# slobodaapl/nvit

Measured on AMD Instinct MI355X. Metric: images/sec (train step) nViT-B/16 224px, higher is better.
Workload: dtype bf16; 1 GPU; nViT-base 224px patches 8/16 T=784 C=768 L=12 H=12, full train step (fwd+bwd+clip+AdamW+renorm), synthetic images, formula weights; per_gpu_batch=128, global_batch=128, parallelism=dp1

## Files before the change

include/nvit_hip.h:

```cpp
#ifndef NVIT_HIP_H
#define NVIT_HIP_H
#include <stdint.h>

#ifdef __cplusplus
extern "C" {
#endif

#define NVIT_OK 0
#define NVIT_EINVAL 1001
#define NVIT_F32 0
#define NVIT_BF16 1
#define NVIT_BF16_F32IN 3

int nvit_version(void);
const char* nvit_last_error(void);

#define NVIT_KID_GEMM_NT 0
#define NVIT_KID_GEMM_TN 1
#define NVIT_KID_ATTN_FWD 2
#define NVIT_KID_ATTN_BWD 3
#define NVIT_KID_ROWOPS 4
#define NVIT_KID_RENORM 5
#define NVIT_KID_SHADOW 6
#define NVIT_KID_PATCHIFY 7
#define NVIT_KID_MISC 8
#define NVIT_KID_GEMM_F32 9
#define NVIT_KID_GEMM_SWIGLU 10
#define NVIT_KID_GEMM_QKNORM 11
#define NVIT_KID_GEMM_SWIGLU_BWD 12
#define NVIT_KID_OPTIM 13
#define NVIT_KID_GEMM_SWIGLU_ACT 14
#define NVIT_KID_COUNT 15
void nvit_prof_enable(int on);
void nvit_prof_select(unsigned mask);
int nvit_prof_collect(double* ms, double* flops, double* bytes, int64_t* launches);
const char* nvit_prof_name(int kid);

#define NVIT_RENORM_ROWS_PER_ITEM 64
#define NVIT_RENORM_COLS_PER_ITEM 64
#define NVIT_RENORM_TALL_ROWS 1152
#define NVIT_RENORM_TALL_COLS_PER_ITEM 32
#define NVIT_RENORM_MAX_ROWS_DIM0 2048
#define NVIT_RENORM_MAX_GRID 2048
int nvit_renorm_weights(const int64_t* table, int n, int total_items, void* stream);

#define NVIT_SHADOW_TILE 64
int nvit_shadow_weights(const int64_t* table, int n, int total_items, int dt, void* stream);

#define NVIT_OPT_TABLE_COLS 10
#define NVIT_OPT_CHUNK 8192
#define NVIT_OPT_ROWS_PER_ITEM 16
#define NVIT_OPT_SLAB_COLS 32
#define NVIT_OPT_SLAB_ROWS 1152
#define NVIT_OPT_TALL_COLS 16
#define NVIT_OPT_TALL_ROWS 2048
#define NVIT_OPT_ROW_COLS 1536
#define NVIT_OPT_WIDE_COLS 2048
#define NVIT_OPT_WIDE_LDS_ROWS 1024
#define NVIT_OPT_MAX_PART 4096
#define NVIT_OPT_MAX_GRID 2048
int nvit_adamw_tick(float* hyper, double beta1, double beta2, void* stream);
int nvit_grad_sqnorm(const int64_t* table, int n, int total_chunks, float* partial, int npart, void* stream);
int nvit_adamw_renorm(const int64_t* table, int n, int total_items, int max_slab_rows, float beta1, float beta2,
                      float eps, double bias_correction1, double bias_correction2, const float* partial, int npart,
                      float max_norm, float* gnorm_out, const float* hyper, void* stream);
int nvit_adamw_tick_guarded(float* hyper, double beta1, double beta2, const float* partial, int npart,
                            float* skip_state, void* stream);
int nvit_adamw_renorm_guarded(const int64_t* table, int n, int total_items, int max_slab_rows, float beta1, float beta2,
                              float eps, const float* partial, int npart, float max_norm, float* gnorm_out,
                              const float* hyper, const float* skip_state, void* stream);
#define NVIT_LR_COSINE 0
#define NVIT_LR_LINEAR 1
#define NVIT_LR_CONSTANT 2
#define NVIT_LR_SCHEDULE_THREADS 256
int nvit_lr_schedule(int64_t* table, int n, const float* lr_scale, int64_t* step, int kind, double lr, double min_lr,
                     double warmup_init, int64_t warmup_iters, int64_t decay_iters, float* last_lr, double* last_lr64,
                     void* stream);

#define NVIT_EMA_TABLE_COLS 5
#define NVIT_EMA_CHUNK 4096
#define NVIT_EMA_MAX_GRID 2048
#define NVIT_EMA_FLAG_COPY 1
#define NVIT_EMA_FLAG_SCALAR 2
int nvit_ema_tick(float* state, double decay, int warmup, const float* skip_state, void* stream);
int nvit_ema_update(const int64_t* table, int n, int total_chunks, const float* state, void* stream);

int nvit_gemm_nt(int dt, const void* A, int lda, const void* B, int ldb, void* C, int ldc, int out_dt,
                 int M, int N, int K, const float* bias, const float* colscale, const float* rowadd,
                 int rowadd_period, int accumulate, void* stream);

#define NVIT_SWIGLU_BWD_TILE_ROWS 256
#define NVIT_SWIGLU_BWD_PART_ROWS 128
int nvit_set_gemm_sched(int dynamic);
int nvit_set_gemm_impl(int nt_impl, int tn_impl);
int nvit_gemm_nt_fusable(int dt, int M, int N, int K);
int nvit_gemm_nt_swiglu_bwd(int dt, const void* A, int lda, const void* B, int ldb, const void* uv, void* duv,
                            float* part, int M, int F, int K, const float* gs, float gscale, void* stream);
int nvit_gemm_nt_swiglu(int dt, const void* A, int lda, const void* B, int ldb, void* uv, void* xm, int M, int F,
                        int K, const float* gs, float gscale, void* stream);
int nvit_gemm_nt_swiglu_act(int dt, const void* A, int lda, const void* B, int ldb, void* xm, int M, int F, int K,
                            const float* gs, float gscale, void* stream);
int nvit_gemm_nt_qknorm(int dt, const void* A, int lda, const void* B, int ldb, int M, int K, int nparts, int part0,
                        const float* sqk, float c_q, float q_prescale, void* qh, void* kh, void* vh, float* rq, float* rk,
                        int T, int H, int d, void* stream);
int nvit_gemm_nt_swiglu_bias(int dt, const void* A, int lda, const void* B, int ldb, void* uv, void* xm, int M, int F,
                             int K, const float* gs, float gscale, const float* bias, void* stream);
int nvit_gemm_nt_swiglu_act_bias(int dt, const void* A, int lda, const void* B, int ldb, void* xm, int M, int F, int K,
                                 const float* gs, float gscale, const float* bias, void* stream);
int nvit_gemm_nt_qknorm_bias(int dt, const void* A, int lda, const void* B, int ldb, int M, int K, int nparts, int part0,
                             const float* sqk, float c_q, float q_prescale, void* qh, void* kh, void* vh, float* rq,
                             float* rk, int T, int H, int d, const float* bias, void* stream);

int nvit_gemm_tn(int dt, const void* A, int lda, const void* B, int ldb, float* G, int ldg, int Mred, int N,
                 int K, int splits, float* ws, int64_t ws_bytes, int perm, int accumulate, void* stream);

#define NVIT_MAX_EMBD 2048
#define NVIT_MAX_PART_BLOCKS 4096
#define NVIT_ROW_WAVES 4
#define NVIT_ROW_GRID_MAX 2048
int nvit_lerp_fwd(int dt, const float* h, const void* y, int y_dt, const float* alpha, float c_a,
                  const float* skip_x, const float* skip, float* out, void* out_lo, int M, int C, void* stream);
int nvit_lerp_bwd_blocks(int dt, int y_dt, int C, int has_add, int has_skip, int accum);
int nvit_lerp_bwd(int dt, const float* dout, const void* dout_add, const float* h, const void* y, int y_dt, const float* alpha,
                  float c_a, const float* skip_x, const float* skip, float* dh, int accum_dh, float* dy,
                  void* dy_lo, float* dskip_x, float* part_dlam, float* part_dskip, int nblk, int M, int C,
                  void* stream);
int nvit_lerp_fwd_gated(int dt, const float* h, const void* y, int y_dt, const float* alpha, float c_a,
                        const float* skip_x, const float* skip, const float* gate, int rows_per_sample, float* out,
                        void* out_lo, int M, int C, void* stream);
int nvit_lerp_bwd_gated_blocks(int dt, int y_dt, int C, int has_add, int has_skip, int accum);
int nvit_lerp_bwd_gated(int dt, const float* dout, const void* dout_add, const float* h, const void* y, int y_dt,
                        const float* alpha, float c_a, const float* skip_x, const float* skip, const float* gate,
                        int rows_per_sample, float* dh, int accum_dh, float* dy, void* dy_lo, float* dskip_x,
                        float* part_dlam, float* part_dskip, int nblk, int M, int C, void* stream);

int nvit_rmsnorm_fwd(const float* x, const float* w, float eps, float* out, float* rstd, int M, int C, void* stream);
int nvit_rmsnorm_bwd(const float* dout, const float* x, const float* w, const float* rstd, float* dx, float* part_dw,
                     int nblk, int M, int C, void* stream);
int nvit_res_rmsnorm_fwd(int dt, const float* a, const void* y, int y_dt, const float* w, float eps, float* out,
                         void* out_lo, float* rstd, int M, int C, void* stream);
int nvit_res_rmsnorm_bwd(int dt, const float* g, const void* g_add, const float* a, const void* y, int y_dt,
                         const float* w, const float* rstd, float* dz, int accum, void* dz_lo, float* part_dw, int nblk,
                         int M, int C, void* stream);
int nvit_res_skip_fwd(int dt, const float* h, const void* y, int y_dt, const float* skip, const float* x, float* out,
                      void* out_lo, int M, int C, void* stream);
int nvit_res_skip_bwd(int dt, const float* dout, const float* h, const void* y, int y_dt, const float* skip,
                      const float* x, float* dh, void* dh_lo, float* dx, float* part_dskip, int nblk, int M, int C,
                      void* stream);
int nvit_res_rmsnorm_fwd_gated(int dt, const float* a, const void* y, int y_dt, const float* w, float eps, const float* gate,
                               int rows_per_sample, float* out, void* out_lo, float* rstd, int M, int C, void* stream);
int nvit_res_rmsnorm_bwd_gated(int dt, const float* g, const void* g_add, const float* a, const void* y, int y_dt,
                               const float* w, const float* rstd, const float* gate, int rows_per_sample, float* dz,
                               int accum, void* dz_lo, float* part_dw, int nblk, int M, int C, void* stream);
int nvit_res_skip_fwd_gated(int dt, const float* h, const void* y, int y_dt, const float* skip, const float* x,
                            const float* gate, int rows_per_sample, float* out, void* out_lo, int M, int C, void* stream);
int nvit_res_skip_bwd_gated(int dt, const float* dout, const float* h, const void* y, int y_dt, const float* skip,
                            const float* x, const float* gate, int rows_per_sample, float* dh, void* dh_lo, float* dx,
                            float* part_dskip, int nblk, int M, int C, void* stream);
int nvit_norm_skip_fwd(const float* src, const float* tgt, const float* skip, float* out, int M, int C, void* stream);
int nvit_norm_skip_bwd(const float* dout, const float* src, const float* tgt, const float* skip, float* dsrc,
                       float* dtgt, float* part_dskip, int nblk, int M, int C, void* stream);

int nvit_qknorm_fwd(int dt, const void* q, int ldq, const void* k, int ldk, const void* v, int ldv,
                    const float* sqk, float c_q, void* qh, void* kh, void* vh, float* rq, float* rk, int B,
                    int T, int H, int d, void* stream);
int nvit_qknorm_bwd(int dt, const void* dqh, const void* dkh, const void* dvh, const void* qh, const void* kh,
                    const float* rq, const float* rk, const float* sqk, float c_q, void* dq, int ldq,
                    void* dk, int ldk, void* dv, int ldv, float* part_dsqk, int nblk, int B, int T, int H,
                    int d, void* stream);

#define NVIT_PAD_HEAD_DIM 128
int nvit_heads_pad_fwd(int dt, const float* q, int ldq, const float* k, int ldk, const float* v, int ldv,
                       const float* sqk, float c_q, void* qh, void* kh, void* vh, float* rq, float* rk,
                       float* sqk_pad, int B, int T, int H, int d, int dp, void* stream);
int nvit_heads_pad_bwd(int dt, const void* dqh, const void* dkh, const void* dvh, const void* qh, const void* kh,
                       const float* rq, const float* rk, const float* sqk, float c_q, void* dq, int ldq,
                       void* dk, int ldk, void* dv, int ldv, float* part_dsqk, int nblk, int B, int T, int H,
                       int d, int dp, void* stream);
int nvit_pad_cols(int dt, const void* src, void* dst, int M, int H, int d, int dp, void* stream);
int nvit_unpad_cols(int dt, const void* src, void* dst, int M, int H, int d, int dp, void* stream);

int nvit_swiglu_fwd(int dt, const void* uv, const float* suv, float gscale, void* x, int M, int F, void* stream);
int nvit_swiglu_bwd(int dt, const void* dx, const void* uv, const float* suv, float gscale, void* duv,
                    float* part_dsuv, int rows_per_blk, int M, int F, void* stream);

int nvit_colsum_reduce(const float* part, int nblk, int N, float* out, int accumulate, int kind, const float* ref,
                       float scale, void* stream);
#define NVIT_COLSUM_REDUCE_MAX_ITEMS 8
int nvit_colsum_reduce_multi(const int64_t* part, const int* nblk, const int64_t* part_b, const int* nblk_b, const int* N,
                             const int64_t* out, const int* accumulate, const int* kind, const int64_t* ref,
                             const float* scale, int n, void* stream);
int nvit_colsum(const void* a, int a_dt, int lda, const void* b, int b_dt, int ldb, int R, int N, int period,
                float* out, int accumulate, float scale, void* stream);
int nvit_cast(const float* src, void* dst, int dt, int64_t n, void* stream);
int nvit_normalize_images(const void* in, int in_is_u8_hwc, float* out, int B, int C, int H, int W, float mean, float std_,
                          void* stream);
#define NVIT_AUG_ROW 8
#define NVIT_AUG_NOPS 15
#define NVIT_AUG_NMAG 10
#define NVIT_AUG_MAX_SIDE 4096
int nvit_augment_draw(const int* policy, int P, uint64_t seed, int64_t* step, int64_t first_index, const int* argtab,
                      int* params, int B, void* stream);
int nvit_augment_apply(const void* in, const int* params, float* out_f32, void* out_u8, void* ws, int64_t ws_bytes, int B,
                       int H, int W, int C, float mean, float std_, void* stream);
#define NVIT_RA_ROW 16
#define NVIT_RA_NCHOICES 15
#define NVIT_RA_SOLARIZE_ADD 15
#define NVIT_RA_NOPS 16
#define NVIT_RA_MAX_LAYERS 4
#define NVIT_RA_ROT_KNOTS 1024
#define NVIT_RA_BILINEAR 0
#define NVIT_RA_BICUBIC 1
#define NVIT_RA_RANDOM 2
int nvit_randaug_draw(uint64_t seed, int64_t* step, int64_t first_index, const double* q, const double* rot, double magnitude,
                      double mstd, double mmax, int increasing, float prob, int interp, double translate_pct, int* params,
                      int B, int num_layers, int H, int W, void* stream);
int nvit_randaug_apply(const void* in, const int* params, float* out_f32, void* out_u8, void* ws, int64_t ws_bytes, int B,
                       int H, int W, int C, int num_layers, int fill0, int fill1, int fill2, float mean, float std_,
                       void* stream);
#define NVIT_MIX_ROW 8
#define NVIT_MIX_KNOTS 1024
int nvit_mix_draw(uint64_t seed, int64_t* step, int64_t first_index, const float* q_mix, const float* q_cut, float prob,
                  float switch_prob, const int64_t* labels, int* table, float* lam, int64_t* y2, int B, int H, int W,
                  void* stream);
int nvit_mix_apply(const float* in, const int* table, float* out, int B, int C, int H, int W, void* stream);
#define NVIT_DROPPATH_MAX_GATES 1048576
int nvit_droppath_draw(uint64_t seed, int64_t* step, int64_t first_index, const float* rates, int scale_by_keep,
                       float* table, int n_layer, int B, void* stream);
#define NVIT_PATCHDROP_MAX_TOKENS 4096
int nvit_patchdrop_draw(uint64_t seed, int64_t* step, int64_t first_index, int* keep, int* slot, int B, int T, int K,
                        void* stream);
int nvit_rows_gather(const float* src0, const float* src1, const int* keep, float* dst0, float* dst1, void* lo0, void* lo1,
                     int lo_dt, int B, int T, int K, int C, void* stream);
int nvit_rows_scatter(const float* d0, const float* d1, const int* slot, float* g0, float* g1, int B, int T, int K, int C,
                      void* stream);
#define NVIT_POS_RESAMPLE_MAX_TAPS 32
#define NVIT_POS_RESAMPLE_MAX_GRID 1024
int nvit_pos_resample_fwd(const float* p0, const float* p1, const int* taps, float* out0, float* out1, int g, int g2, int C,
                          void* stream);
int nvit_pos_resample_bwd(const float* d0, const float* d1, const int* taps_t, float* g0, float* g1, int g, int g2, int C,
                          void* stream);
#define NVIT_CROP_ROW 8
#define NVIT_CROP_KNOTS 1024
#define NVIT_CROP_ATTEMPTS 10
#define NVIT_CROP_MAX_SRC 2048
#define NVIT_CROP_MAX_BATCH 65535
#define NVIT_CROP_BILINEAR 0
#define NVIT_CROP_BICUBIC 1
int nvit_crop_draw(uint64_t seed, int64_t* step, int64_t first_index, const double* aspect, double scale0, double scale1,
                   double ratio_min, double ratio_max, float hflip, int* table, int B, int Hs, int Ws, void* stream);
int64_t nvit_crop_ws_bytes(int B, int Hs, int Ws, int C, int size, int interp);
int nvit_crop_apply(const void* in, const int* table, void* out, void* ws, int64_t ws_bytes, int B, int Hs, int Ws, int C,
                    int size, int interp, void* stream);
#define NVIT_ERASE_ROW 8
#define NVIT_ERASE_KNOTS 1024
#define NVIT_ERASE_CONST 0
#define NVIT_ERASE_PIXEL 1
int nvit_erase_draw(uint64_t seed, int64_t* step, int64_t first_index, const double* aspect, double area0, double area1,
                    float prob, int* table, int B, int H, int W, void* stream);
int nvit_erase_apply(const float* in, const int* table, const float* q, float* out, int mode, int B, int C, int H, int W,
                     void* stream);
int nvit_scale_cols(const float* a, int lda, const float* s, float c, void* out, int out_dt, int ldo, int R, int N,
                    void* stream);

int nvit_attn_fwd(int dt, int impl, const void* qh, const void* kh, const void* vh, float scale, void* o, float* lse,
                  int B, int H, int Tq, int Tk, int d, void* stream);
int nvit_attn_fwd_bounded(int dt, int impl, const void* qh, const void* kh, const void* vh, float scale, const float* sqk,
                          float c_q, float q_prescale, void* o, float* lse, int B, int H, int Tq, int Tk, int d,
                          void* stream);
int nvit_attn_bwd(int dt, int impl, const void* dout, const void* qh, const void* kh, const void* vh, const void* o,
                  const float* lse, float scale, void* dqh, void* dkh, void* dvh, float* delta, int B, int H,
                  int Tq, int Tk, int d, void* stream);

#define NVIT_ATTN_BWD_PART_ROWS 128
int nvit_attn_bwd_qknorm(int dt, const void* dout, const void* qh, const void* kh, const void* vh, const void* o,
                         const float* lse, float scale, const float* rq, const float* rk, const float* sqk, float c_q,
                         float q_prescale, void* dq, int ldq, void* dk, void* dv, int ldkv, float* part_q, float* part_k,
                         float* delta, int B, int H, int Tq, int Tk, int d, void* stream);

// ... 77 lines not shown
```

nvit_amd/_lib.py:

```python
from __future__ import annotations

import ctypes as C
import os
import re

_HERE = os.path.dirname(os.path.abspath(__file__))
LIB_PATH = os.environ.get("NVIT_LIB") or os.path.join(_HERE, "libnvit_hip.so")
HEADER_PATH = os.path.join(os.path.dirname(_HERE), "include", "nvit_hip.h")


def _header_constants() -> dict:
    try:
        with open(HEADER_PATH) as f:
            return {name: int(value) for name, value in re.findall(r"#define NVIT_(\w+)\s+(-?\d+)", f.read())}
    except OSError as e:
        raise ImportError(f"nvit_amd: cannot read the C header that holds the kernels' layout constants: {e}") from None


HEADER = _header_constants()


def const(name: str) -> int:
    if name not in HEADER:
        raise ImportError(f"nvit_amd: {HEADER_PATH} has no integer `#define NVIT_{name}`")
    return HEADER[name]


F32, BF16, BF16_F32IN = 0, 1, 3
KID_NAMES = ["gemm_nt", "gemm_tn", "attn_fwd", "attn_bwd", "rowops", "renorm", "shadow", "patchify", "misc", "gemm_f32",
             "gemm_swiglu", "gemm_qknorm", "gemm_swiglu_bwd", "optim", "gemm_swiglu_act"]
RENORM_ROWS_PER_ITEM = const("RENORM_ROWS_PER_ITEM")
RENORM_COLS_PER_ITEM = const("RENORM_COLS_PER_ITEM")
RENORM_TALL_ROWS = const("RENORM_TALL_ROWS")
RENORM_TALL_COLS_PER_ITEM = const("RENORM_TALL_COLS_PER_ITEM")
RENORM_MAX_ROWS_DIM0 = const("RENORM_MAX_ROWS_DIM0")
MAX_EMBD = const("MAX_EMBD")
ATTN_HEADS_MAX_H = const("ATTN_HEADS_MAX_H")

_vp, _i, _f, _i64 = C.c_void_p, C.c_int, C.c_float, C.c_int64

SIGNATURES = {
    "nvit_version": [],
    "nvit_last_error": [],
    "nvit_prof_enable": [_i],
    "nvit_prof_select": [C.c_uint],
    "nvit_prof_collect": [_vp, _vp, _vp, _vp],
    "nvit_prof_name": [_i],
    "nvit_renorm_weights": [_vp, _i, _i, _vp],
    "nvit_shadow_weights": [_vp, _i, _i, _i, _vp],
    "nvit_grad_sqnorm": [_vp, _i, _i, _vp, _i, _vp],
    "nvit_adamw_renorm": [_vp, _i, _i, _i, _f, _f, _f, C.c_double, C.c_double, _vp, _i, _f, _vp, _vp, _vp],
    "nvit_adamw_tick": [_vp, C.c_double, C.c_double, _vp],
    "nvit_adamw_tick_guarded": [_vp, C.c_double, C.c_double, _vp, _i, _vp, _vp],
    "nvit_adamw_renorm_guarded": [_vp, _i, _i, _i, _f, _f, _f, _vp, _i, _f, _vp, _vp, _vp, _vp],
    "nvit_lr_schedule": [_vp, _i, _vp, _vp, _i, C.c_double, C.c_double, C.c_double, _i64, _i64, _vp, _vp, _vp],
    "nvit_ema_tick": [_vp, C.c_double, _i, _vp, _vp],
    "nvit_ema_update": [_vp, _i, _i, _vp, _vp],
    "nvit_set_gemm_sched": [_i],
    "nvit_set_gemm_impl": [_i, _i],
    "nvit_ce_loss": [_vp, _vp, _vp, _vp, _vp, _i, _i, _vp],
    "nvit_ce_loss_soft": [_vp, _vp, _vp, _vp, _f, _vp, _vp, _vp, _i, _i, _vp],
    "nvit_eval_metrics": [_vp, _vp, _vp, _i, _i, _vp],
    "nvit_gemm_nt": [_i, _vp, _i, _vp, _i, _vp, _i, _i, _i, _i, _i, _vp, _vp, _vp, _i, _i, _vp],
    "nvit_gemm_nt_fusable": [_i, _i, _i, _i],
    "nvit_gemm_nt_swiglu": [_i, _vp, _i, _vp, _i, _vp, _vp, _i, _i, _i, _vp, _f, _vp],
    "nvit_gemm_nt_swiglu_act": [_i, _vp, _i, _vp, _i, _vp, _i, _i, _i, _vp, _f, _vp],
    "nvit_gemm_nt_swiglu_bwd": [_i, _vp, _i, _vp, _i, _vp, _vp, _vp, _i, _i, _i, _vp, _f, _vp],
    "nvit_gemm_nt_qknorm": [_i, _vp, _i, _vp, _i, _i, _i, _i, _i, _vp, _f, _f, _vp, _vp, _vp, _vp, _vp, _i, _i, _i, _vp],
    "nvit_gemm_nt_swiglu_bias": [_i, _vp, _i, _vp, _i, _vp, _vp, _i, _i, _i, _vp, _f, _vp, _vp],
    "nvit_gemm_nt_swiglu_act_bias": [_i, _vp, _i, _vp, _i, _vp, _i, _i, _i, _vp, _f, _vp, _vp],
    "nvit_gemm_nt_qknorm_bias": [_i, _vp, _i, _vp, _i, _i, _i, _i, _i, _vp, _f, _f, _vp, _vp, _vp, _vp, _vp, _i, _i, _i, _vp,
                                 _vp],
    "nvit_gemm_tn": [_i, _vp, _i, _vp, _i, _vp, _i, _i, _i, _i, _i, _vp, _i64, _i, _i, _vp],
    "nvit_lerp_fwd": [_i, _vp, _vp, _i, _vp, _f, _vp, _vp, _vp, _vp, _i, _i, _vp],
    "nvit_lerp_bwd_blocks": [_i, _i, _i, _i, _i, _i],
    "nvit_lerp_bwd": [_i, _vp, _vp, _vp, _vp, _i, _vp, _f, _vp, _vp, _vp, _i, _vp, _vp, _vp, _vp, _vp, _i, _i, _i, _vp],
    "nvit_lerp_fwd_gated": [_i, _vp, _vp, _i, _vp, _f, _vp, _vp, _vp, _i, _vp, _vp, _i, _i, _vp],
    "nvit_lerp_bwd_gated_blocks": [_i, _i, _i, _i, _i, _i],
    "nvit_lerp_bwd_gated": [_i, _vp, _vp, _vp, _vp, _i, _vp, _f, _vp, _vp, _vp, _i, _vp, _i, _vp, _vp, _vp, _vp, _vp, _i, _i,
                            _i, _vp],
    "nvit_norm_skip_fwd": [_vp, _vp, _vp, _vp, _i, _i, _vp],
    "nvit_norm_skip_bwd": [_vp, _vp, _vp, _vp, _vp, _vp, _vp, _i, _i, _i, _vp],
    "nvit_qknorm_fwd": [_i, _vp, _i, _vp, _i, _vp, _i, _vp, _f, _vp, _vp, _vp, _vp, _vp, _i, _i, _i, _i, _vp],
    "nvit_qknorm_bwd": [_i, _vp, _vp, _vp, _vp, _vp, _vp, _vp, _vp, _f, _vp, _i, _vp, _i, _vp, _i, _vp, _i, _i, _i,
                        _i, _i, _vp],
    "nvit_heads_pad_fwd": [_i, _vp, _i, _vp, _i, _vp, _i, _vp, _f, _vp, _vp, _vp, _vp, _vp, _vp, _i, _i, _i, _i, _i, _vp],
    "nvit_heads_pad_bwd": [_i, _vp, _vp, _vp, _vp, _vp, _vp, _vp, _vp, _f, _vp, _i, _vp, _i, _vp, _i, _vp, _i, _i, _i,
                           _i, _i, _i, _vp],
    "nvit_pad_cols": [_i, _vp, _vp, _i, _i, _i, _i, _vp],
    "nvit_unpad_cols": [_i, _vp, _vp, _i, _i, _i, _i, _vp],
    "nvit_swiglu_fwd": [_i, _vp, _vp, _f, _vp, _i, _i, _vp],
    "nvit_swiglu_bwd": [_i, _vp, _vp, _vp, _f, _vp, _vp, _i, _i, _i, _vp],
    "nvit_colsum_reduce_multi": [_vp, _vp, _vp, _vp, _vp, _vp, _vp, _vp, _vp, _vp, _i, _vp],
    "nvit_colsum_reduce": [_vp, _i, _i, _vp, _i, _i, _vp, _f, _vp],
    "nvit_colsum": [_vp, _i, _i, _vp, _i, _i, _i, _i, _i, _vp, _i, _f, _vp],
    "nvit_cast": [_vp, _vp, _i, _i64, _vp],
    "nvit_normalize_images": [_vp, _i, _vp, _i, _i, _i, _i, _f, _f, _vp],
    "nvit_augment_draw": [_vp, _i, C.c_uint64, _vp, _i64, _vp, _vp, _i, _vp],
    "nvit_augment_apply": [_vp, _vp, _vp, _vp, _vp, _i64, _i, _i, _i, _i, _f, _f, _vp],
    "nvit_randaug_draw": [C.c_uint64, _vp, _i64, _vp, _vp, C.c_double, C.c_double, C.c_double, _i, _f, _i, C.c_double, _vp,
                          _i, _i, _i, _i, _vp],
    "nvit_randaug_apply": [_vp, _vp, _vp, _vp, _vp, _i64, _i, _i, _i, _i, _i, _i, _i, _i, _f, _f, _vp],
    "nvit_mix_draw": [C.c_uint64, _vp, _i64, _vp, _vp, _f, _f, _vp, _vp, _vp, _vp, _i, _i, _i, _vp],
    "nvit_mix_apply": [_vp, _vp, _vp, _i, _i, _i, _i, _vp],
    "nvit_droppath_draw": [C.c_uint64, _vp, _i64, _vp, _i, _vp, _i, _i, _vp],
    "nvit_patchdrop_draw": [C.c_uint64, _vp, _i64, _vp, _vp, _i, _i, _i, _vp],
    "nvit_rows_gather": [_vp, _vp, _vp, _vp, _vp, _vp, _vp, _i, _i, _i, _i, _i, _vp],
    "nvit_rows_scatter": [_vp, _vp, _vp, _vp, _vp, _i, _i, _i, _i, _vp],
    "nvit_pos_resample_fwd": [_vp, _vp, _vp, _vp, _vp, _i, _i, _i, _vp],
    "nvit_pos_resample_bwd": [_vp, _vp, _vp, _vp, _vp, _i, _i, _i, _vp],
    "nvit_crop_draw": [C.c_uint64, _vp, _i64, _vp, C.c_double, C.c_double, C.c_double, C.c_double, _f, _vp, _i, _i, _i, _vp],
    "nvit_crop_ws_bytes": [_i, _i, _i, _i, _i, _i],
    "nvit_crop_apply": [_vp, _vp, _vp, _vp, _i64, _i, _i, _i, _i, _i, _i, _vp],
    "nvit_erase_draw": [C.c_uint64, _vp, _i64, _vp, C.c_double, C.c_double, _f, _vp, _i, _i, _i, _vp],
    "nvit_erase_apply": [_vp, _vp, _vp, _vp, _i, _i, _i, _i, _i, _vp],
    "nvit_scale_cols": [_vp, _i, _vp, _f, _vp, _i, _i, _i, _i, _vp],
    "nvit_attn_fwd": [_i, _i, _vp, _vp, _vp, _f, _vp, _vp, _i, _i, _i, _i, _i, _vp],
    "nvit_attn_fwd_bounded": [_i, _i, _vp, _vp, _vp, _f, _vp, _f, _f, _vp, _vp, _i, _i, _i, _i, _i, _vp],
    "nvit_attn_bwd": [_i, _i, _vp, _vp, _vp, _vp, _vp, _vp, _f, _vp, _vp, _vp, _vp, _i, _i, _i, _i, _i, _vp],
    "nvit_attn_bwd_qknorm": [_i, _vp, _vp, _vp, _vp, _vp, _vp, _f, _vp, _vp, _vp, _f, _f, _vp, _i, _vp, _vp, _i, _vp, _vp,
                             _vp, _i, _i, _i, _i, _i, _vp],
    "nvit_attn_heads_fwd": [_i, _vp, _i, _vp, _vp, _i, _vp, _f, _f, _vp, _vp, _i, _i, _i, _vp],
    "nvit_attn_heads_bwd": [_i, _vp, _vp, _i, _vp, _vp, _i, _vp, _f, _f, _vp, _vp, _i, _vp, _vp, _i, _vp, _i, _i, _i, _i,
                            _vp],
    "nvit_im2col": [_i, _vp, _vp, _vp, _i, _i, _i, _i, _i, _vp],
    "nvit_patch_embed_kp": [_i],
    "nvit_patch_embed_fwd": [_vp, _vp, _vp, _vp, _vp, _vp, _vp, _vp, _vp, _vp, _vp, _vp, _vp, _i, _i, _i, _i, _i, _i, _vp],
    "nvit_pool_ln_fwd": [_i, _vp, _vp, _vp, _f, _vp, _vp, _vp, _vp, _vp, _i, _i, _i, _i, _vp],
    "nvit_pool_ln_bwd": [_vp, _vp, _vp, _vp, _vp, _vp, _vp, _i, _i, _i, _i, _vp],
    "nvit_som_bmu": [_vp, _vp, _vp, _i64, _i, _i, _vp, _vp],
    "nvit_gather_rows": [_vp, _vp, _vp, _i64, _i, _vp],
    "nvit_scatter_rows": [_vp, _vp, _vp, _i64, _i, _i, _vp],
    "nvit_onehot": [_vp, _vp, _i64, _i, _vp],
    "nvit_rmsnorm_fwd": [_vp, _vp, _f, _vp, _vp, _i, _i, _vp],
    "nvit_rmsnorm_bwd": [_vp, _vp, _vp, _vp, _vp, _vp, _i, _i, _i, _vp],
    "nvit_res_rmsnorm_fwd": [_i, _vp, _vp, _i, _vp, _f, _vp, _vp, _vp, _i, _i, _vp],
    "nvit_res_rmsnorm_bwd": [_i, _vp, _vp, _vp, _vp, _i, _vp, _vp, _vp, _i, _vp, _vp, _i, _i, _i, _vp],
    "nvit_res_skip_fwd": [_i, _vp, _vp, _i, _vp, _vp, _vp, _vp, _i, _i, _vp],
    "nvit_res_skip_bwd": [_i, _vp, _vp, _vp, _i, _vp, _vp, _vp, _vp, _vp, _vp, _i, _i, _i, _vp],
    "nvit_res_rmsnorm_fwd_gated": [_i, _vp, _vp, _i, _vp, _f, _vp, _i, _vp, _vp, _vp, _i, _i, _vp],
    "nvit_res_rmsnorm_bwd_gated": [_i, _vp, _vp, _vp, _vp, _i, _vp, _vp, _vp, _i, _vp, _i, _vp, _vp, _i, _i, _i, _vp],
    "nvit_res_skip_fwd_gated": [_i, _vp, _vp, _i, _vp, _vp, _vp, _i, _vp, _vp, _i, _i, _vp],
    "nvit_res_skip_bwd_gated": [_i, _vp, _vp, _vp, _i, _vp, _vp, _vp, _i, _vp, _vp, _vp, _vp, _i, _i, _i, _vp],
    "nvit_som_update": [_vp, _vp, _vp, _f, _f, _i, _i, _i, _vp, _vp, _i, _i, _i, _vp],
    "nvit_som_update_dev": [_vp, _vp, _vp, _vp, _f, _i, _i, _i, _vp, _vp, _i, _i, _i, _vp],
    "nvit_cos_consistency_fwd": [_vp, _vp, _vp, _vp, _i, _vp, _i64, _i, _vp],
    "nvit_cos_consistency_bwd": [_vp, _vp, _vp, _vp, _vp, _vp, _i64, _i, _vp],
    "nvit_huber_fwd": [_vp, _vp, _vp, _i, _vp, _i64, _vp],
    "nvit_huber_bwd": [_vp, _vp, _vp, _vp, _vp, _i64, _vp],
    "nvit_som_smooth_fwd": [_vp, _vp, _vp, _vp, _vp, _i64, _i, _i, _i, _vp],
    "nvit_som_smooth_bwd": [_vp, _vp, _vp, _vp, _vp, _i, _i64, _i, _i, _i, _vp],
    "nvit_recon_bwd": [_i, _vp, _vp, _vp, _vp, _i, _i, _i, _i, _vp],
    "nvit_recon_loss": [_vp, _vp, _vp, _i, _vp, _i, _i, _i, _i, _vp],
    "nvit_xgmi_chunk": [_i64, _i],
    "nvit_xgmi_reduce_scatter": [_vp, _i, _i, _i64, _f, _vp],
    "nvit_xgmi_all_gather": [_vp, _i, _i, _i64, _vp],
    "nvit_xgmi_flag_bytes": [_i],
    "nvit_xgmi_flags_alloc": [_i, _vp, _vp],
    "nvit_xgmi_flags_open": [_vp, _vp],
    "nvit_xgmi_flags_close": [_vp],
    "nvit_xgmi_flags_free": [_vp],
    "nvit_xgmi_flags_error": [_vp, _i, _vp, _vp],
    "nvit_xgmi_reduce_scatter_sync": [_vp, _vp, _i, _i, _i, _i, C.c_uint, _i64, _i64, _f, _vp],
    "nvit_xgmi_all_gather_sync": [_vp, _vp, _i, _i, _i, _i, C.c_uint, _i64, _i64, _vp],
    "nvit_xgmi_wait_gathered": [_vp, _i, _i, _i, _vp, _vp, _i, _vp, _vp],
    "nvit_xgmi_set_timeout": [C.c_double],
    "nvit_xgmi_errword_alloc": [_vp, _vp],
    "nvit_xgmi_errword_free": [_vp],
    "nvit_set_attn_dkv_asm": [_i],
}
_RESTYPES = {"nvit_last_error": C.c_char_p, "nvit_prof_name": C.c_char_p, "nvit_prof_enable": None, "nvit_prof_select": None,
             "nvit_xgmi_chunk": C.c_int64, "nvit_xgmi_flag_bytes": C.c_int64, "nvit_crop_ws_bytes": C.c_int64}

_lib = None


def load() -> C.CDLL:
    global _lib
    if _lib is not None:
        return _lib
    if not os.path.exists(LIB_PATH):
        raise RuntimeError(
            f"nvit_amd: {LIB_PATH} not found. Build it with `python -c 'import __graft_entry__ as g; g.build()'` "
            "(hipcc --offload-arch=gfx950). There is no CPU fallback for the nViT hot path.")
    lib = C.CDLL(LIB_PATH)
    for name, args in SIGNATURES.items():
        fn = getattr(lib, name)
        fn.argtypes = args
        fn.restype = _RESTYPES.get(name, C.c_int)
    _lib = lib
    return lib


def check(rc: int, what: str) -> None:
    if rc != 0:
        msg = load().nvit_last_error()
        raise RuntimeError(f"{what} failed (code {rc}): {msg.decode() if msg else ''}")
```

nvit_amd/csrc/rowops.hip:

```cpp
#include "dispatch.h"

namespace {

constexpr int ROW_WAVES = NVIT_ROW_WAVES;
static_assert(ROW_WAVES * 64 == 256, "the row kernels launch 256 threads");

template <int NV>
struct RowVec {
  f32x4 v[NV];
};

template <int NV, typename T>
__device__ __forceinline__ void row_load(RowVec<NV>& r, const T* p, int C, int lane) {
#pragma unroll
  for (int i = 0; i < NV; ++i) {
    const int c = (i * 64 + lane) * 4;
    r.v[i] = c < C ? load4<T>(p + c) : (f32x4){0.f, 0.f, 0.f, 0.f};
  }
}
template <int NV, typename T>
__device__ __forceinline__ void row_store(const RowVec<NV>& r, T* p, int C, int lane) {
#pragma unroll
  for (int i = 0; i < NV; ++i) {
    const int c = (i * 64 + lane) * 4;
    if (c < C) store4<T>(p + c, r.v[i]);
  }
}
template <int NV>
__device__ __forceinline__ float row_dot(const RowVec<NV>& a, const RowVec<NV>& b) {
  float s = 0.f;
#pragma unroll
  for (int i = 0; i < NV; ++i) s += a.v[i][0] * b.v[i][0] + a.v[i][1] * b.v[i][1] + a.v[i][2] * b.v[i][2] + a.v[i][3] * b.v[i][3];
  return wave_sum(s);
}

template <int NV>
__device__ __forceinline__ void row_load_f32_nt(RowVec<NV>& r, const float* p, int C, int lane) {
#pragma unroll
  for (int i = 0; i < NV; ++i) {
    const int c = (i * 64 + lane) * 4;
    r.v[i] = c < C ? __builtin_nontemporal_load(reinterpret_cast<const f32x4*>(p + c)) : (f32x4){0.f, 0.f, 0.f, 0.f};
  }
}

struct LerpFwdArgs {
  const float* h;
  const void* y;
  const float* alpha;
  float c_a;
  const float* skip_x;
  const float* skip;
  float* out;
  void* out_lo;
  int M, C;
  const float* gate;
  int T;
};

__device__ __forceinline__ float row_gate(const float* gate, int m, int T) {
  typedef const __attribute__((address_space(4))) float* cfloat_p;
  return ((cfloat_p)gate)[__builtin_amdgcn_readfirstlane(m) / T];
}

template <int NV, typename TY, typename TL, bool GATED>
__global__ __launch_bounds__(256) void lerp_fwd_kernel(LerpFwdArgs a) {
  const int lane = threadIdx.x & 63, wid = threadIdx.x >> 6;
  RowVec<NV> lam;
  row_load<NV, float>(lam, a.alpha, a.C, lane);
#pragma unroll
  for (int i = 0; i < NV; ++i)
#pragma unroll
    for (int e = 0; e < 4; ++e) lam.v[i][e] = fabsf(lam.v[i][e] * a.c_a);
  const float skip = a.skip_x ? a.skip[0] : 0.f;
  for (int m = blockIdx.x * ROW_WAVES + wid; m < a.M; m += gridDim.x * ROW_WAVES) {
    RowVec<NV> x, y, r, xs;
    row_load_f32_nt<NV>(x, a.h + (size_t)m * a.C, a.C, lane);
#pragma unroll
    for (int i = 0; i < NV; ++i) {
      const int c = (i * 64 + lane) * 4;
      if constexpr (sizeof(TY) == 2) {
        uint2 raw = make_uint2(0u, 0u);
        if (c < a.C) {
          typedef unsigned int u32x2_ __attribute__((ext_vector_type(2)));
          raw = __builtin_bit_cast(uint2, __builtin_nontemporal_load(reinterpret_cast<const u32x2_*>(reinterpret_cast<const TY*>(a.y) + (size_t)m * a.C + c)));
        }
        const bf16x4 b4 = __builtin_bit_cast(bf16x4, raw);
        y.v[i] = (f32x4){(float)b4[0], (float)b4[1], (float)b4[2], (float)b4[3]};
      } else {
        y.v[i] = c < a.C ? __builtin_nontemporal_load(reinterpret_cast<const f32x4*>(reinterpret_cast<const float*>(a.y) + (size_t)m * a.C + c)) : (f32x4){0.f, 0.f, 0.f, 0.f};
      }
    }
    if (a.skip_x) row_load_f32_nt<NV>(xs, a.skip_x + (size_t)m * a.C, a.C, lane);
    float gt = 1.0f;
    if constexpr (GATED) gt = row_gate(a.gate, m, a.T);
    const float rsx = 1.0f / sqrtf(row_dot<NV>(x, x));
    const float rsy = 1.0f / sqrtf(row_dot<NV>(y, y));
#pragma unroll
    for (int i = 0; i < NV; ++i) {
      const f32x4 av = x.v[i] * rsx, bv = y.v[i] * rsy;
      if constexpr (GATED) r.v[i] = av + (lam.v[i] * gt) * (bv - av);
      else r.v[i] = av + lam.v[i] * (bv - av);
    }
    const float rsr = 1.0f / sqrtf(row_dot<NV>(r, r));
#pragma unroll
    for (int i = 0; i < NV; ++i) r.v[i] = r.v[i] * rsr;
    if (a.skip_x) {
#pragma unroll
      for (int i = 0; i < NV; ++i) r.v[i] = r.v[i] * skip + xs.v[i];
      const float rst = 1.0f / sqrtf(row_dot<NV>(r, r));
#pragma unroll
      for (int i = 0; i < NV; ++i) r.v[i] = r.v[i] * rst;
    }
#pragma unroll
    for (int i = 0; i < NV; ++i) {
      const int c = (i * 64 + lane) * 4;
      if (c < a.C) __builtin_nontemporal_store(r.v[i], reinterpret_cast<f32x4*>(a.out + (size_t)m * a.C + c));
    }
    if (a.out_lo) row_store<NV, TL>(r, reinterpret_cast<TL*>(a.out_lo) + (size_t)m * a.C, a.C, lane);
  }
}

struct LerpBwdArgs {
  const float* dout;
  const bf16* dout_add;
  const float* h;
  const void* y;
  const float* alpha;
  float c_a;
  const float* skip_x;
  const float* skip;
  float* dh;
  int accum_dh;
  float* dy;
  void* dy_lo;
  float* dskip_x;
  float* part_dlam;
  float* part_dskip;
  int M, C;
  const float* gate;
  int T;
};

template <int NV>
__device__ __forceinline__ float dot4(const f32x4& a, const f32x4& b) {
  return a[0] * b[0] + a[1] * b[1] + a[2] * b[2] + a[3] * b[3];
}

template <int NV, typename TY, typename TL, bool ADD, bool SKIP, bool ACCUM, bool GATED>
__global__ __launch_bounds__(256, 1) void lerp_bwd_kernel(LerpBwdArgs a) {
  const int lane = threadIdx.x & 63, wid = threadIdx.x >> 6;
  RowVec<NV> lam, dlam;
  row_load<NV, float>(lam, a.alpha, a.C, lane);
#pragma unroll
  for (int i = 0; i < NV; ++i) {
    dlam.v[i] = (f32x4){0.f, 0.f, 0.f, 0.f};
#pragma unroll
    for (int e = 0; e < 4; ++e) lam.v[i][e] = fabsf(lam.v[i][e] * a.c_a);
  }
  const float skip = SKIP ? a.skip[0] : 0.f;
  float dskip_acc = 0.f;
  for (int m = blockIdx.x * ROW_WAVES + wid; m < a.M; m += gridDim.x * ROW_WAVES) {
    RowVec<NV> av, bv, g, t, old;
    uint2 ga[NV];
    const size_t ro = (size_t)m * a.C;
    row_load_f32_nt<NV>(av, a.h + ro, a.C, lane);
    row_load<NV, TY>(bv, reinterpret_cast<const TY*>(a.y) + ro, a.C, lane);
    row_load_f32_nt<NV>(g, a.dout + ro, a.C, lane);
    if constexpr (ADD) {
#pragma unroll
      for (int i = 0; i < NV; ++i) {
        const int c = (i * 64 + lane) * 4;
        ga[i] = c < a.C ? *reinterpret_cast<const uint2*>(a.dout_add + ro + c) : make_uint2(0u, 0u);
      }
    }
    if constexpr (SKIP) row_load_f32_nt<NV>(t, a.skip_x + ro, a.C, lane);
    float gt = 1.0f;
    if constexpr (GATED) gt = row_gate(a.gate, m, a.T);
#define NVIT_LAM(i_) (GATED ? lam.v[i_] * gt : lam.v[i_])
    if constexpr (ADD) {
#pragma unroll
      for (int i = 0; i < NV; ++i) {
        const bf16x4 q = __builtin_bit_cast(bf16x4, ga[i]);
        g.v[i] += (f32x4){(float)q[0], (float)q[1], (float)q[2], (float)q[3]};
      }
    }
    const float rsx = 1.0f / sqrtf(row_dot<NV>(av, av));
    const float rsy = 1.0f / sqrtf(row_dot<NV>(bv, bv));
    if constexpr (ACCUM) row_load<NV, float>(old, a.dh + ro, a.C, lane);
    float ss = 0.f;
#pragma unroll
    for (int i = 0; i < NV; ++i) {
      av.v[i] = av.v[i] * rsx;
      bv.v[i] = bv.v[i] * rsy;
      const f32x4 ou = av.v[i] + NVIT_LAM(i) * (bv.v[i] - av.v[i]);
      ss += dot4<NV>(ou, ou);
    }
    const float rsr = 1.0f / sqrtf(wave_sum(ss));
#define NVIT_LERP_O(i_) ((av.v[i_] + NVIT_LAM(i_) * (bv.v[i_] - av.v[i_])) * rsr)
    if constexpr (SKIP) {
      float st = 0.f;
#pragma unroll
      for (int i = 0; i < NV; ++i) {
        t.v[i] = NVIT_LERP_O(i) * skip + t.v[i];
        st += dot4<NV>(t.v[i], t.v[i]);
      }
      const float rst = 1.0f / sqrtf(wave_sum(st));
      float tg = 0.f;
#pragma unroll
      for (int i = 0; i < NV; ++i) {
        t.v[i] = t.v[i] * rst;
        tg += dot4<NV>(t.v[i], g.v[i]);
      }
      tg = wave_sum(tg);
      float dso = 0.f;
#pragma unroll
      for (int i = 0; i < NV; ++i) {
        g.v[i] = (g.v[i] - t.v[i] * tg) * rst;
        dso += dot4<NV>(g.v[i], NVIT_LERP_O(i));
      }
      row_store<NV, float>(g, a.dskip_x + ro, a.C, lane);
      dskip_acc += wave_sum(dso);
#pragma unroll
      for (int i = 0; i < NV; ++i) g.v[i] = g.v[i] * skip;
    }
    float og = 0.f;
#pragma unroll
    for (int i = 0; i < NV; ++i) og += dot4<NV>(NVIT_LERP_O(i), g.v[i]);
    og = wave_sum(og);
    float ada = 0.f, bdb = 0.f;
#pragma unroll
    for (int i = 0; i < NV; ++i) {
      g.v[i] = (g.v[i] - NVIT_LERP_O(i) * og) * rsr;
      dlam.v[i] += (GATED ? g.v[i] * gt : g.v[i]) * (bv.v[i] - av.v[i]);
      const f32x4 db = NVIT_LAM(i) * g.v[i];
      ada += dot4<NV>(av.v[i], g.v[i] - db);
      bdb += dot4<NV>(bv.v[i], db);
    }
#undef NVIT_LERP_O
    ada = wave_sum(ada);
    bdb = wave_sum(bdb);
#pragma unroll
    for (int i = 0; i < NV; ++i) {
      const int c = (i * 64 + lane) * 4;
      const f32x4 db = NVIT_LAM(i) * g.v[i];
      f32x4 dh = ((g.v[i] - db) - av.v[i] * ada) * rsx;
      const f32x4 dy = (db - bv.v[i] * bdb) * rsy;
      if constexpr (ACCUM) dh += old.v[i];
      if (c < a.C) {
        store4<float>(a.dh + ro + c, dh);
        if (a.dy) store4<float>(a.dy + ro + c, dy);
        if (a.dy_lo) store4<TL>(reinterpret_cast<TL*>(a.dy_lo) + ro + c, dy);
      }
    }
#undef NVIT_LAM
  }
  const size_t prow = (size_t)blockIdx.x * ROW_WAVES + wid;
  row_store<NV, float>(dlam, a.part_dlam + prow * a.C, a.C, lane);
  if (SKIP && lane == 0) a.part_dskip[prow] = dskip_acc;
}

template <int NV>
__global__ __launch_bounds__(256) void norm_skip_fwd_kernel(const float* src, const float* tgt, const float* skip,
                                                             float* out, int M, int C) {
  const int lane = threadIdx.x & 63, wid = threadIdx.x >> 6;
  const float sk = skip[0];
  for (int m = blockIdx.x * ROW_WAVES + wid; m < M; m += gridDim.x * ROW_WAVES) {
    RowVec<NV> a, b;
    row_load<NV, float>(a, src + (size_t)m * C, C, lane);
    if (tgt) {
      row_load<NV, float>(b, tgt + (size_t)m * C, C, lane);
#pragma unroll
      for (int i = 0; i < NV; ++i) a.v[i] = a.v[i] * sk + b.v[i];
    } else {
#pragma unroll
      for (int i = 0; i < NV; ++i) a.v[i] = a.v[i] * sk;
    }
    const float rs = 1.0f / sqrtf(row_dot<NV>(a, a));
#pragma unroll
    for (int i = 0; i < NV; ++i) a.v[i] = a.v[i] * rs;
    row_store<NV, float>(a, out + (size_t)m * C, C, lane);
  }
}

template <int NV>
__global__ __launch_bounds__(256) void norm_skip_bwd_kernel(const float* dout, const float* src, const float* tgt,
                                                             const float* skip, float* dsrc, float* dtgt,
                                                             float* part_dskip, int M, int C) {
  __shared__ float red[ROW_WAVES];
  const int lane = threadIdx.x & 63, wid = threadIdx.x >> 6;
  const float sk = skip[0];
  float acc = 0.f;
  for (int m = blockIdx.x * ROW_WAVES + wid; m < M; m += gridDim.x * ROW_WAVES) {
    RowVec<NV> a, b, g;
    row_load<NV, float>(a, src + (size_t)m * C, C, lane);
    if (tgt) {
      row_load<NV, float>(b, tgt + (size_t)m * C, C, lane);
    } else {
#pragma unroll
      for (int i = 0; i < NV; ++i) b.v[i] = (f32x4){0.f, 0.f, 0.f, 0.f};
    }
    row_load<NV, float>(g, dout + (size_t)m * C, C, lane);
#pragma unroll
    for (int i = 0; i < NV; ++i) b.v[i] = a.v[i] * sk + b.v[i];
    const float rs = 1.0f / sqrtf(row_dot<NV>(b, b));
#pragma unroll
    for (int i = 0; i < NV; ++i) b.v[i] = b.v[i] * rs;
    const float og = row_dot<NV>(b, g);
#pragma unroll
    for (int i = 0; i < NV; ++i) g.v[i] = (g.v[i] - b.v[i] * og) * rs;
    acc += row_dot<NV>(g, a);
    if (dtgt) row_store<NV, float>(g, dtgt + (size_t)m * C, C, lane);
#pragma unroll
    for (int i = 0; i < NV; ++i) g.v[i] = g.v[i] * sk;
    row_store<NV, float>(g, dsrc + (size_t)m * C, C, lane);
  }
  if (lane == 0) red[wid] = acc;
  __syncthreads();
  if (threadIdx.x == 0) part_dskip[blockIdx.x] = red[0] + red[1] + red[2] + red[3];
}

constexpr int PAD_D = NVIT_PAD_HEAD_DIM;

struct QkArgs {
  const void *q, *k, *v;
  int ldq, ldk, ldv;
  const float* sqk;
  float c_q;
  void *qh, *kh, *vh;
  float *rq, *rk;
  float* sqk_pad;
  int B, T, H, d;
};

__device__ __forceinline__ float dot4_fma(f32x4 a, f32x4 b) {
  return __builtin_fmaf(a[3], b[3], __builtin_fmaf(a[2], b[2], __builtin_fmaf(a[0], b[0], a[1] * b[1])));
}
__device__ __forceinline__ float dot4_sum(f32x4 a, f32x4 b) {
#pragma clang fp contract(off)
  return a[0] * b[0] + a[1] * b[1] + a[2] * b[2] + a[3] * b[3];
}

template <int NV, typename TI, typename T, bool NORM>
__global__ __launch_bounds__(256) void qknorm_fwd_kernel(QkArgs a) {
  const int lane = threadIdx.x & 63, wid = threadIdx.x >> 6;
  const int C = a.H * a.d, M = a.B * a.T, G = a.d >> 2;
  RowVec<NV> s;
  if constexpr (NORM) {
    row_load<NV, float>(s, a.sqk, C, lane);
#pragma unroll
    for (int i = 0; i < NV; ++i) s.v[i] = s.v[i] * a.c_q;
  }
  for (int m = blockIdx.x * ROW_WAVES + wid; m < M; m += gridDim.x * ROW_WAVES) {
    const int b = m / a.T, t = m % a.T;
    RowVec<NV> q, k, v;
    row_load<NV, TI>(q, reinterpret_cast<const TI*>(a.q) + (size_t)m * a.ldq, C, lane);
    row_load<NV, TI>(k, reinterpret_cast<const TI*>(a.k) + (size_t)m * a.ldk, C, lane);
    row_load<NV, TI>(v, reinterpret_cast<const TI*>(a.v) + (size_t)m * a.ldv, C, lane);
#pragma unroll
    for (int i = 0; i < NV; ++i) {
      const int c = (i * 64 + lane) * 4;
      const int h = c / a.d, j = c % a.d;
      const size_t dst = (((size_t)b * a.H + h) * a.T + t) * a.d + j;
      if constexpr (!NORM) {
        if (c < C) {
          store4<T>(reinterpret_cast<T*>(a.qh) + dst, q.v[i]);
          store4<T>(reinterpret_cast<T*>(a.kh) + dst, k.v[i]);
          store4<T>(reinterpret_cast<T*>(a.vh) + dst, v.v[i]);
        }
      } else {
        const float sq = group_sum_dyn(dot4_sum(q.v[i], q.v[i]), G), sk = group_sum_dyn(dot4_fma(k.v[i], k.v[i]), G);
        if (c < C) {
          const float rq = 1.0f / sqrtf(sq), rk = 1.0f / sqrtf(sk);
          store4<T>(reinterpret_cast<T*>(a.qh) + dst, q.v[i] * rq * s.v[i]);
          store4<T>(reinterpret_cast<T*>(a.kh) + dst, k.v[i] * rk * s.v[i]);
          store4<T>(reinterpret_cast<T*>(a.vh) + dst, v.v[i]);
          if (j == 0) {
            a.rq[(size_t)m * a.H + h] = rq;
            a.rk[(size_t)m * a.H + h] = rk;
          }
        }
      }
    }
  }
}

template <typename T, bool NORM>
__global__ __launch_bounds__(256) void heads_pad_fwd_kernel(QkArgs a) {
  const int lane = threadIdx.x & 63, wid = threadIdx.x >> 6;
  const int M = a.B * a.T, HP = a.H * PAD_D;
  const float *aq = reinterpret_cast<const float*>(a.q), *ak = reinterpret_cast<const float*>(a.k),
              *av = reinterpret_cast<const float*>(a.v);
  const f32x4 z = {0.f, 0.f, 0.f, 0.f};
  if constexpr (NORM) {
// ... 503 lines not shown
  for (int i = 0; i < NV; ++i) dw.v[i] = (f32x4){0.f, 0.f, 0.f, 0.f};
  for (int m = blockIdx.x * ROW_WAVES + wid; m < a.M; m += gridDim.x * ROW_WAVES) {
    RowVec<NV> z, g;
    row_load<NV, float>(z, a.a + (size_t)m * a.C, a.C, lane);
    row_load_f32_nt<NV>(g, a.g + (size_t)m * a.C, a.C, lane);
    float gt = 1.0f;
    if constexpr (GATED) gt = row_gate(a.gate, m, a.T);
    if constexpr (HAS_Y) {
      RowVec<NV> y;
      row_load<NV, TY>(y, reinterpret_cast<const TY*>(a.y) + (size_t)m * a.C, a.C, lane);
      if constexpr (GATED) {
#pragma unroll
        for (int i = 0; i < NV; ++i) y.v[i] = y.v[i] * gt;
      }
#pragma unroll
      for (int i = 0; i < NV; ++i) z.v[i] = z.v[i] + y.v[i];
    }
    if constexpr (ADD) {
      RowVec<NV> ad;
      row_load<NV, TL>(ad, reinterpret_cast<const TL*>(a.g_add) + (size_t)m * a.C, a.C, lane);
#pragma unroll
      for (int i = 0; i < NV; ++i) g.v[i] = g.v[i] + ad.v[i];
    }
    const float rs = a.rstd[m];
#pragma unroll
    for (int i = 0; i < NV; ++i) {
      z.v[i] = z.v[i] * rs;
      dw.v[i] += g.v[i] * z.v[i];
      g.v[i] = g.v[i] * wv.v[i];
    }
    const float mean = row_dot<NV>(g, z) / (float)a.C;
#pragma unroll
    for (int i = 0; i < NV; ++i) g.v[i] = (g.v[i] - z.v[i] * mean) * rs;
    float* dz = a.dz + (size_t)m * a.C;
    if (a.accum) {
      RowVec<NV> old;
      row_load<NV, float>(old, dz, a.C, lane);
#pragma unroll
      for (int i = 0; i < NV; ++i) g.v[i] = g.v[i] + old.v[i];
    }
    row_store<NV, float>(g, dz, a.C, lane);
    if constexpr (GATED) {
#pragma unroll
      for (int i = 0; i < NV; ++i) g.v[i] = g.v[i] * gt;
    }
    if (a.dz_lo) row_store<NV, TL>(g, reinterpret_cast<TL*>(a.dz_lo) + (size_t)m * a.C, a.C, lane);
  }
  row_store<NV, float>(dw, a.part_dw + ((size_t)blockIdx.x * ROW_WAVES + wid) * a.C, a.C, lane);
}

struct ResSkipArgs {
  const float* dout;
  const float* h;
  const void* y;
  const float* skip;
  const float* x;
  float* out;
  void* out_lo;
  float* dh;
  float* part_dskip;
  int M, C;
  const float* gate;
  int T;
};

template <int NV, typename TY, typename TL, bool GATED>
__global__ __launch_bounds__(256) void res_skip_fwd_kernel(ResSkipArgs a) {
  const int lane = threadIdx.x & 63, wid = threadIdx.x >> 6;
  const float sk = a.skip[0];
  for (int m = blockIdx.x * ROW_WAVES + wid; m < a.M; m += gridDim.x * ROW_WAVES) {
    RowVec<NV> r, y, x;
    row_load<NV, float>(r, a.h + (size_t)m * a.C, a.C, lane);
    row_load<NV, TY>(y, reinterpret_cast<const TY*>(a.y) + (size_t)m * a.C, a.C, lane);
    row_load<NV, float>(x, a.x + (size_t)m * a.C, a.C, lane);
    if constexpr (GATED) {
      const float gt = row_gate(a.gate, m, a.T);
#pragma unroll
      for (int i = 0; i < NV; ++i) y.v[i] = y.v[i] * gt;
    }
#pragma unroll
    for (int i = 0; i < NV; ++i) r.v[i] = (r.v[i] + y.v[i]) * sk + x.v[i];
    const float rs = 1.0f / sqrtf(row_dot<NV>(r, r));
#pragma unroll
    for (int i = 0; i < NV; ++i) r.v[i] = r.v[i] * rs;
    row_store<NV, float>(r, a.out + (size_t)m * a.C, a.C, lane);
    if (a.out_lo) row_store<NV, TL>(r, reinterpret_cast<TL*>(a.out_lo) + (size_t)m * a.C, a.C, lane);
  }
}

template <int NV, typename TY, typename TL, bool GATED>
__global__ __launch_bounds__(256) void res_skip_bwd_kernel(ResSkipArgs a) {
  const int lane = threadIdx.x & 63, wid = threadIdx.x >> 6;
  const float sk = a.skip[0];
  float acc = 0.f;
  for (int m = blockIdx.x * ROW_WAVES + wid; m < a.M; m += gridDim.x * ROW_WAVES) {
    RowVec<NV> s, y, r, g;
    row_load<NV, float>(s, a.h + (size_t)m * a.C, a.C, lane);
    row_load<NV, TY>(y, reinterpret_cast<const TY*>(a.y) + (size_t)m * a.C, a.C, lane);
    row_load<NV, float>(r, a.x + (size_t)m * a.C, a.C, lane);
    row_load_f32_nt<NV>(g, a.dout + (size_t)m * a.C, a.C, lane);
    float gt = 1.0f;
    if constexpr (GATED) {
      gt = row_gate(a.gate, m, a.T);
#pragma unroll
      for (int i = 0; i < NV; ++i) y.v[i] = y.v[i] * gt;
    }
#pragma unroll
    for (int i = 0; i < NV; ++i) {
      s.v[i] = s.v[i] + y.v[i];
      r.v[i] = s.v[i] * sk + r.v[i];
    }
    const float rs = 1.0f / sqrtf(row_dot<NV>(r, r));
#pragma unroll
    for (int i = 0; i < NV; ++i) r.v[i] = r.v[i] * rs;
    const float og = row_dot<NV>(r, g);
#pragma unroll
    for (int i = 0; i < NV; ++i) g.v[i] = (g.v[i] - r.v[i] * og) * rs;
    acc += row_dot<NV>(g, s);
    row_store<NV, float>(g, a.out + (size_t)m * a.C, a.C, lane);
#pragma unroll
    for (int i = 0; i < NV; ++i) g.v[i] = g.v[i] * sk;
    row_store<NV, float>(g, a.dh + (size_t)m * a.C, a.C, lane);
    if constexpr (GATED) {
#pragma unroll
      for (int i = 0; i < NV; ++i) g.v[i] = g.v[i] * gt;
    }
    if (a.out_lo) row_store<NV, TL>(g, reinterpret_cast<TL*>(a.out_lo) + (size_t)m * a.C, a.C, lane);
  }
  if (lane == 0) a.part_dskip[(size_t)blockIdx.x * ROW_WAVES + wid] = acc;
}

int row_grid(int M) {
  const int blocks = cdiv(M, ROW_WAVES);
  return blocks > NVIT_ROW_GRID_MAX ? NVIT_ROW_GRID_MAX : blocks;
}

}


template <typename F>
static auto with_row_types(int C, int y_dt, int dt, F&& f) {
  return with_row_vecs<8>(C, [&](auto nv) {
    return with_elem(y_dt, [&](auto ty) { return with_elem(dt, [&](auto tl) { return f(nv, ty, tl); }); });
  });
}

template <typename F>
static auto with_in_out_elems(int dt, F&& f) {
  if (dt == NVIT_F32) return f(type_tag<float>{}, type_tag<float>{});
  if (dt == NVIT_BF16) return f(type_tag<bf16>{}, type_tag<bf16>{});
  return f(type_tag<float>{}, type_tag<bf16>{});
}

static auto lerp_bwd_select(int C, int y_dt, int dt, bool has_add, bool has_skip, bool accum) -> void (*)(LerpBwdArgs) {
  return with_row_types(C, y_dt, dt, [&](auto nv, auto ty, auto tl) {
    return with_bool(has_add, [&](auto add) {
      return with_bool(has_skip, [&](auto skip) {
        return with_bool(accum, [&](auto acc) {
          return &lerp_bwd_kernel<nv, tag_t<decltype(ty)>, tag_t<decltype(tl)>, add, skip, acc, false>;
        });
      });
    });
  });
}

static auto lerp_bwd_gated_select(int C, int y_dt, int dt, bool has_add, bool mlp_half) -> void (*)(LerpBwdArgs) {
  return with_row_types(C, y_dt, dt, [&](auto nv, auto ty, auto tl) {
    return with_bool(has_add, [&](auto add) {
      using TY = tag_t<decltype(ty)>;
      using TL = tag_t<decltype(tl)>;
      if (mlp_half) return &lerp_bwd_kernel<nv, TY, TL, add, true, false, true>;
      return &lerp_bwd_kernel<nv, TY, TL, add, false, true, true>;
    });
  });
}

static bool gate_args_ok(const float* gate, int rows_per_sample, int M) {
  return gate && rows_per_sample > 0 && M % rows_per_sample == 0;
}

extern "C" int nvit_lerp_fwd(int dt, const float* h, const void* y, int y_dt, const float* alpha, float c_a,
                             const float* skip_x, const float* skip, float* out, void* out_lo, int M, int C,
                             void* stream) {
  NVIT_REQUIRE(C % 4 == 0 && C <= NVIT_MAX_EMBD && M > 0, "lerp_fwd: C=%d must be a multiple of 4 and <= %d", C, NVIT_MAX_EMBD);
  NVIT_REQUIRE(!skip_x || skip, "lerp_fwd: skip_x without skip");
  LerpFwdArgs a{h, y, alpha, c_a, skip_x, skip, out, out_lo, M, C, nullptr, 1};
  hipStream_t s = (hipStream_t)stream;
  const int grid = row_grid(M);
  ProfScope ps(NVIT_KID_ROWOPS, 0.0, (double)M * C * (skip_x ? 16.0 : 12.0), s);
  const auto kernel = with_row_types(C, y_dt, dt, [](auto nv, auto ty, auto tl) {
    return &lerp_fwd_kernel<nv, tag_t<decltype(ty)>, tag_t<decltype(tl)>, false>;
  });
  launch(kernel, dim3(grid), dim3(256), 0, s, a);
  NVIT_CHECK_LAUNCH("lerp_fwd");
  return NVIT_OK;
}

extern "C" int nvit_lerp_fwd_gated(int dt, const float* h, const void* y, int y_dt, const float* alpha, float c_a,
                                   const float* skip_x, const float* skip, const float* gate, int rows_per_sample,
                                   float* out, void* out_lo, int M, int C, void* stream) {
  NVIT_REQUIRE(C % 4 == 0 && C <= NVIT_MAX_EMBD && M > 0, "lerp_fwd_gated: C=%d must be a multiple of 4 and <= %d", C, NVIT_MAX_EMBD);
  NVIT_REQUIRE(!skip_x || skip, "lerp_fwd_gated: skip_x without skip");
  NVIT_REQUIRE(gate_args_ok(gate, rows_per_sample, M), "lerp_fwd_gated: gate missing, or M=%d is no multiple of rows_per_sample=%d", M, rows_per_sample);
  LerpFwdArgs a{h, y, alpha, c_a, skip_x, skip, out, out_lo, M, C, gate, rows_per_sample};
  hipStream_t s = (hipStream_t)stream;
  ProfScope ps(NVIT_KID_ROWOPS, 0.0, (double)M * C * (skip_x ? 16.0 : 12.0) + 4.0 * M, s);
  const auto kernel = with_row_types(C, y_dt, dt, [](auto nv, auto ty, auto tl) {
    return &lerp_fwd_kernel<nv, tag_t<decltype(ty)>, tag_t<decltype(tl)>, true>;
  });
  launch(kernel, dim3(row_grid(M)), dim3(256), 0, s, a);
  NVIT_CHECK_LAUNCH("lerp_fwd_gated");
  return NVIT_OK;
}

static int resident_blocks(void (*kernel)(LerpBwdArgs)) {
  int per_cu = 0;
  if (hipOccupancyMaxActiveBlocksPerMultiprocessor(&per_cu, kernel, 256, 0) != hipSuccess || per_cu < 1) return 0;
  return per_cu * nvit_num_cu();
}

extern "C" int nvit_lerp_bwd_blocks(int dt, int y_dt, int C, int has_add, int has_skip, int accum) {
  if (C % 4 != 0 || C <= 0 || C > NVIT_MAX_EMBD) return 0;
  const int n = resident_blocks(lerp_bwd_select(C, y_dt, dt, has_add, has_skip, accum));
  return n > NVIT_MAX_PART_BLOCKS ? NVIT_MAX_PART_BLOCKS : n;
}

extern "C" int nvit_lerp_bwd_gated_blocks(int dt, int y_dt, int C, int has_add, int has_skip, int accum) {
  if (C % 4 != 0 || C <= 0 || C > NVIT_MAX_EMBD || (has_skip != 0) == (accum != 0)) return 0;
  const int n = resident_blocks(lerp_bwd_gated_select(C, y_dt, dt, has_add, has_skip != 0));
  return n > NVIT_MAX_PART_BLOCKS ? NVIT_MAX_PART_BLOCKS : n;
}

extern "C" int nvit_lerp_bwd(int dt, const float* dout, const void* dout_add, const float* h, const void* y, int y_dt, const float* alpha,
                             float c_a, const float* skip_x, const float* skip, float* dh, int accum_dh, float* dy,
                             void* dy_lo, float* dskip_x, float* part_dlam, float* part_dskip, int nblk, int M,
                             int C, void* stream) {
  NVIT_REQUIRE(C % 4 == 0 && C <= NVIT_MAX_EMBD && M > 0, "lerp_bwd: C=%d must be a multiple of 4 and <= %d", C, NVIT_MAX_EMBD);
  NVIT_REQUIRE(nblk > 0 && nblk <= NVIT_MAX_PART_BLOCKS, "lerp_bwd: nblk out of range");
  NVIT_REQUIRE(!skip_x || (skip && dskip_x && part_dskip), "lerp_bwd: skip buffers missing");
  LerpBwdArgs a{dout, (const bf16*)dout_add, h, y, alpha, c_a, skip_x, skip, dh, accum_dh, dy, dy_lo, dskip_x, part_dlam, part_dskip, M, C, nullptr, 1};
  hipStream_t s = (hipStream_t)stream;
  const double lb_bytes = (double)M * C * (4.0 + 4.0 + (y_dt == NVIT_F32 ? 4.0 : 2.0) + 4.0 + (dy ? 4.0 : 0.0) + (dy_lo ? (dt == NVIT_F32 ? 4.0 : 2.0) : 0.0) +
                                           (skip_x ? 8.0 : 0.0) + (accum_dh ? 4.0 : 0.0) + (dout_add ? 2.0 : 0.0));
  ProfScope ps(NVIT_KID_ROWOPS, 0.0, lb_bytes, s);
  launch(lerp_bwd_select(C, y_dt, dt, dout_add != nullptr, skip_x != nullptr, accum_dh != 0), dim3(nblk), dim3(256), 0, s, a);
  NVIT_CHECK_LAUNCH("lerp_bwd");
  return NVIT_OK;
}

extern "C" int nvit_lerp_bwd_gated(int dt, const float* dout, const void* dout_add, const float* h, const void* y, int y_dt,
                                   const float* alpha, float c_a, const float* skip_x, const float* skip,
                                   const float* gate, int rows_per_sample, float* dh, int accum_dh, float* dy, void* dy_lo,
                                   float* dskip_x, float* part_dlam, float* part_dskip, int nblk, int M, int C,
                                   void* stream) {
  NVIT_REQUIRE(C % 4 == 0 && C <= NVIT_MAX_EMBD && M > 0, "lerp_bwd_gated: C=%d must be a multiple of 4 and <= %d", C, NVIT_MAX_EMBD);
  NVIT_REQUIRE(nblk > 0 && nblk <= NVIT_MAX_PART_BLOCKS, "lerp_bwd_gated: nblk out of range");
  NVIT_REQUIRE(!skip_x || (skip && dskip_x && part_dskip), "lerp_bwd_gated: skip buffers missing");
  NVIT_REQUIRE(gate_args_ok(gate, rows_per_sample, M), "lerp_bwd_gated: gate missing, or M=%d is no multiple of rows_per_sample=%d", M, rows_per_sample);
  NVIT_REQUIRE((skip_x != nullptr) != (accum_dh != 0),
               "lerp_bwd_gated: built for the two calls of the block chain, skip_x without accum_dh or accum_dh without skip_x");
  LerpBwdArgs a{dout, (const bf16*)dout_add, h, y, alpha, c_a, skip_x, skip, dh, accum_dh, dy, dy_lo, dskip_x, part_dlam, part_dskip, M, C, gate, rows_per_sample};
  hipStream_t s = (hipStream_t)stream;
  const double lb_bytes = (double)M * C * (4.0 + 4.0 + (y_dt == NVIT_F32 ? 4.0 : 2.0) + 4.0 + (dy ? 4.0 : 0.0) + (dy_lo ? (dt == NVIT_F32 ? 4.0 : 2.0) : 0.0) +
                                           (skip_x ? 8.0 : 0.0) + (accum_dh ? 4.0 : 0.0) + (dout_add ? 2.0 : 0.0)) + 4.0 * M;
  ProfScope ps(NVIT_KID_ROWOPS, 0.0, lb_bytes, s);
  launch(lerp_bwd_gated_select(C, y_dt, dt, dout_add != nullptr, skip_x != nullptr), dim3(nblk), dim3(256), 0, s, a);
  NVIT_CHECK_LAUNCH("lerp_bwd_gated");
  return NVIT_OK;
}

extern "C" int nvit_norm_skip_fwd(const float* src, const float* tgt, const float* skip, float* out, int M, int C,
                                  void* stream) {
  NVIT_REQUIRE(C % 4 == 0 && C <= NVIT_MAX_EMBD && M > 0, "norm_skip_fwd: C=%d must be a multiple of 4 and <= %d", C, NVIT_MAX_EMBD);
  hipStream_t s = (hipStream_t)stream;
  const int grid = row_grid(M);
  with_row_vecs<8>(C, [&](auto nv) { launch(norm_skip_fwd_kernel<nv>, dim3(grid), dim3(256), 0, s, src, tgt, skip, out, M, C); });
  NVIT_CHECK_LAUNCH("norm_skip_fwd");
  return NVIT_OK;
}

extern "C" int nvit_norm_skip_bwd(const float* dout, const float* src, const float* tgt, const float* skip, float* dsrc,
                                  float* dtgt, float* part_dskip, int nblk, int M, int C, void* stream) {
  NVIT_REQUIRE(C % 4 == 0 && C <= NVIT_MAX_EMBD && M > 0 && nblk > 0 && nblk <= NVIT_MAX_PART_BLOCKS, "norm_skip_bwd: bad arguments");
  hipStream_t s = (hipStream_t)stream;
  with_row_vecs<8>(C, [&](auto nv) {
    launch(norm_skip_bwd_kernel<nv>, dim3(nblk), dim3(256), 0, s, dout, src, tgt, skip, dsrc, dtgt, part_dskip, M, C);
  });
  NVIT_CHECK_LAUNCH("norm_skip_bwd");
  return NVIT_OK;
}

extern "C" int nvit_rmsnorm_fwd(const float* x, const float* w, float eps, float* out, float* rstd, int M, int C,
                                void* stream) {
  NVIT_REQUIRE(C % 4 == 0 && C <= NVIT_MAX_EMBD && M > 0, "rmsnorm_fwd: C=%d must be a multiple of 4 and <= %d", C, NVIT_MAX_EMBD);
  hipStream_t s = (hipStream_t)stream;
  const int grid = row_grid(M);
  with_row_vecs<8>(C, [&](auto nv) { launch(rmsnorm_fwd_kernel<nv>, dim3(grid), dim3(256), 0, s, x, w, eps, out, rstd, M, C); });
  NVIT_CHECK_LAUNCH("rmsnorm_fwd");
  return NVIT_OK;
}

extern "C" int nvit_rmsnorm_bwd(const float* dout, const float* x, const float* w, const float* rstd, float* dx,
                                float* part_dw, int nblk, int M, int C, void* stream) {
  NVIT_REQUIRE(C % 4 == 0 && C <= NVIT_MAX_EMBD && M > 0 && nblk > 0 && nblk <= NVIT_MAX_PART_BLOCKS, "rmsnorm_bwd: bad arguments");
  hipStream_t s = (hipStream_t)stream;
  with_row_vecs<8>(C, [&](auto nv) {
    launch(rmsnorm_bwd_kernel<nv>, dim3(nblk), dim3(256), 0, s, dout, x, w, rstd, dx, part_dw, M, C);
  });
  NVIT_CHECK_LAUNCH("rmsnorm_bwd");
  return NVIT_OK;
}

extern "C" int nvit_res_rmsnorm_fwd(int dt, const float* a, const void* y, int y_dt, const float* w, float eps, float* out,
                                    void* out_lo, float* rstd, int M, int C, void* stream) {
  NVIT_REQUIRE(C % 4 == 0 && C <= NVIT_MAX_EMBD && M > 0, "res_rmsnorm_fwd: C=%d must be a multiple of 4 and <= %d", C, NVIT_MAX_EMBD);
  NVIT_REQUIRE(dt == NVIT_F32 || dt == NVIT_BF16, "res_rmsnorm_fwd: bad dt %d", dt);
  NVIT_REQUIRE(!y || y_dt == NVIT_F32 || y_dt == NVIT_BF16, "res_rmsnorm_fwd: bad y_dt %d", y_dt);
  ResRmsFwdArgs ar{a, y, w, eps, out, out_lo, rstd, M, C, nullptr, 1};
  hipStream_t s = (hipStream_t)stream;
  const int grid = row_grid(M);
  ProfScope ps(NVIT_KID_ROWOPS, 0.0, (double)M * C * (8.0 + (y ? (y_dt == NVIT_F32 ? 4.0 : 2.0) : 0.0) +
                                                       (out_lo ? (dt == NVIT_F32 ? 4.0 : 2.0) : 0.0)), s);
  const auto kernel = with_row_vecs<8>(C, [&](auto nv) {
    return with_elem(dt, [&](auto tl) {
      using TL = tag_t<decltype(tl)>;
      if (!y) return &res_rmsnorm_fwd_kernel<nv, float, TL, false, false>;
      return with_elem(y_dt, [&](auto ty) { return &res_rmsnorm_fwd_kernel<nv, tag_t<decltype(ty)>, TL, true, false>; });
    });
  });
  launch(kernel, dim3(grid), dim3(256), 0, s, ar);
  NVIT_CHECK_LAUNCH("res_rmsnorm_fwd");
  return NVIT_OK;
}

extern "C" int nvit_res_rmsnorm_bwd(int dt, const float* g, const void* g_add, const float* a, const void* y, int y_dt,
                                    const float* w, const float* rstd, float* dz, int accum, void* dz_lo, float* part_dw,
                                    int nblk, int M, int C, void* stream) {
  NVIT_REQUIRE(C % 4 == 0 && C <= NVIT_MAX_EMBD && M > 0, "res_rmsnorm_bwd: C=%d must be a multiple of 4 and <= %d", C, NVIT_MAX_EMBD);
  NVIT_REQUIRE(nblk > 0 && nblk <= NVIT_MAX_PART_BLOCKS, "res_rmsnorm_bwd: nblk out of range");
  NVIT_REQUIRE(dt == NVIT_F32 || dt == NVIT_BF16, "res_rmsnorm_bwd: bad dt %d", dt);
  NVIT_REQUIRE(!y || y_dt == NVIT_F32 || y_dt == NVIT_BF16, "res_rmsnorm_bwd: bad y_dt %d", y_dt);
  ResRmsBwdArgs ar{g, g_add, a, y, w, rstd, dz, accum, dz_lo, part_dw, M, C, nullptr, 1};
  hipStream_t s = (hipStream_t)stream;
  const double tl = dt == NVIT_F32 ? 4.0 : 2.0;
  ProfScope ps(NVIT_KID_ROWOPS, 0.0, (double)M * C * (12.0 + (y ? (y_dt == NVIT_F32 ? 4.0 : 2.0) : 0.0) +
                                                       (g_add ? tl : 0.0) + (accum ? 4.0 : 0.0) + (dz_lo ? tl : 0.0)), s);
  const auto kernel = with_row_vecs<8>(C, [&](auto nv) {
    return with_elem(dt, [&](auto tlo) {
      return with_bool(g_add != nullptr, [&](auto add) {
        using TL = tag_t<decltype(tlo)>;
        if (!y) return &res_rmsnorm_bwd_kernel<nv, float, TL, false, add, false>;
        return with_elem(y_dt, [&](auto ty) { return &res_rmsnorm_bwd_kernel<nv, tag_t<decltype(ty)>, TL, true, add, false>; });
      });
    });
  });
  launch(kernel, dim3(nblk), dim3(256), 0, s, ar);
  NVIT_CHECK_LAUNCH("res_rmsnorm_bwd");
  return NVIT_OK;
}

extern "C" int nvit_res_skip_fwd(int dt, const float* h, const void* y, int y_dt, const float* skip, const float* x,
                                 float* out, void* out_lo, int M, int C, void* stream) {
  NVIT_REQUIRE(C % 4 == 0 && C <= NVIT_MAX_EMBD && M > 0, "res_skip_fwd: C=%d must be a multiple of 4 and <= %d", C, NVIT_MAX_EMBD);
  NVIT_REQUIRE(dt == NVIT_F32 || dt == NVIT_BF16, "res_skip_fwd: bad dt %d", dt);
  NVIT_REQUIRE(y && (y_dt == NVIT_F32 || y_dt == NVIT_BF16), "res_skip_fwd: y missing or bad y_dt %d", y_dt);
  ResSkipArgs ar{nullptr, h, y, skip, x, out, out_lo, nullptr, nullptr, M, C, nullptr, 1};
  hipStream_t s = (hipStream_t)stream;
  const int grid = row_grid(M);
  ProfScope ps(NVIT_KID_ROWOPS, 0.0, (double)M * C * (12.0 + (y_dt == NVIT_F32 ? 4.0 : 2.0) +
                                                       (out_lo ? (dt == NVIT_F32 ? 4.0 : 2.0) : 0.0)), s);
  const auto kernel = with_row_types(C, y_dt, dt, [](auto nv, auto ty, auto tl) {
    return &res_skip_fwd_kernel<nv, tag_t<decltype(ty)>, tag_t<decltype(tl)>, false>;
  });
  launch(kernel, dim3(grid), dim3(256), 0, s, ar);
  NVIT_CHECK_LAUNCH("res_skip_fwd");
  return NVIT_OK;
}

extern "C" int nvit_res_skip_bwd(int dt, const float* dout, const float* h, const void* y, int y_dt, const float* skip,
                                 const float* x, float* dh, void* dh_lo, float* dx, float* part_dskip, int nblk, int M,
                                 int C, void* stream) {
  NVIT_REQUIRE(C % 4 == 0 && C <= NVIT_MAX_EMBD && M > 0, "res_skip_bwd: C=%d must be a multiple of 4 and <= %d", C, NVIT_MAX_EMBD);
  NVIT_REQUIRE(nblk > 0 && nblk <= NVIT_MAX_PART_BLOCKS, "res_skip_bwd: nblk out of range");
  NVIT_REQUIRE(dt == NVIT_F32 || dt == NVIT_BF16, "res_skip_bwd: bad dt %d", dt);
  NVIT_REQUIRE(y && (y_dt == NVIT_F32 || y_dt == NVIT_BF16), "res_skip_bwd: y missing or bad y_dt %d", y_dt);
  ResSkipArgs ar{dout, h, y, skip, x, dx, dh_lo, dh, part_dskip, M, C, nullptr, 1};
  hipStream_t s = (hipStream_t)stream;
  ProfScope ps(NVIT_KID_ROWOPS, 0.0, (double)M * C * (20.0 + (y_dt == NVIT_F32 ? 4.0 : 2.0) +
                                                       (dh_lo ? (dt == NVIT_F32 ? 4.0 : 2.0) : 0.0)), s);
  const auto kernel = with_row_types(C, y_dt, dt, [](auto nv, auto ty, auto tl) {
    return &res_skip_bwd_kernel<nv, tag_t<decltype(ty)>, tag_t<decltype(tl)>, false>;
  });
  launch(kernel, dim3(nblk), dim3(256), 0, s, ar);
  NVIT_CHECK_LAUNCH("res_skip_bwd");
  return NVIT_OK;
}

extern "C" int nvit_res_rmsnorm_fwd_gated(int dt, const float* a, const void* y, int y_dt, const float* w, float eps,
                                          const float* gate, int rows_per_sample, float* out, void* out_lo, float* rstd,
// ... 355 lines not shown
```

nvit_amd/model.py:

```python
from __future__ import annotations

import dataclasses
import math
import os
from typing import Dict, Optional, Tuple

import torch
from torch import nn

from . import ops, resample
from ._lib import ATTN_HEADS_MAX_H, BF16, BF16_F32IN, F32, MAX_EMBD
from .config import ViTConfig
from .kohonen import CosConsistencyFn, HuberFn, KohonenMap, MapSmoothnessFn

Tensor = torch.Tensor
HEAD_DIMS = (32, 64, 128)
PADDED_HEAD_DIMS = (72, 80, 88, 104)


def _dt_from_precision(p: str) -> int:
    if p == "fp32":
        return F32
    if p == "bf16":
        return BF16
# ... 171 lines not shown
        ops.colsum_big(dy_lo, M, N, g, False)
    else:
        part = torch.empty((512, N), device=dy_lo.device, dtype=torch.float32)
        ops.colsum(dy_lo, M, N, part, False, period=512)
        ops.colsum_reduce(part, g, False, kind=2)
    return g


def _lo(rt: _Runtime, x: Tensor, x_lo: Tensor) -> Tensor:
    return x.detach() if rt.dt == F32 else x_lo


def _take_carry(rt: "_Runtime", idx: int, chained: bool, dout: Tensor):
    c, rt.carry = rt.carry, None
    if c is None:
        return dout, None
    want, dx, add = c
    if not chained or want != idx:
        raise RuntimeError("nvit_amd: pending q/k/v data gradient was not consumed by the block it was produced for")
    if dout.data_ptr() != dx.data_ptr():
        return dout + add.float(), None
    return dout, add


RMS_EPS = 1e-6


def _lean() -> bool:
    return not torch.is_grad_enabled()


def _dims(rt: _Runtime, M: int):
    cfg = rt.model.config
    T = rt.n_tokens
    return M // T, T, cfg.n_embd, cfg.n_head, cfg.n_embd // cfg.n_head, M


def _qkv_cols(ts, C: int):
    if len(ts) == 1:
        qkv, = ts
        return qkv, 3 * C, qkv[:, C:], qkv[:, 2 * C:], 3 * C
    q, kv = ts
    return q, C, kv, kv[:, C:], 2 * C


def _attn_fwd(rt: _Runtime, impl: int, srcs, sqk: Optional[Tensor], c_q: float, scale: float, dims,
              lean: bool = False):
    B, T, C, H, d, M = dims
    dt, sh = rt.dt, rt.sh
    heads = rt.model.config.flash_attn
    dp = ops.PAD_HEAD_DIM if d in PADDED_HEAD_DIMS else d
    sqk_a = sqk
    if not heads and impl == 1 and d == 64 and C % 256 == 0 and ops.fusable(dt, M, srcs[0][2] * C, C):
        route = "fused"
        qpre = ops.attn_q_prescale(d) if sqk is not None else ops.LOG2E / math.sqrt(d)
        bufs = ops.qk_buffers(dt, B, T, H, d, srcs[0][0].device, norm=sqk is not None)
        part0 = 0
        for A, w, n in srcs:
            ops.gemm_nt_qknorm(A, sh[w + ".W"], M, C, n, part0, sqk, c_q, B, T, H, d, bufs,
                               q_prescale=(qpre if part0 == 0 else 1.0), bias=sh.get(w + ".b"))
            part0 += n
    else:
        projs = [ops.gemm_nt(A, sh[w + ".W"], M, n * C, C, out_dtype=torch.float32, bias=sh.get(w + ".b"))
                 for A, w, n in srcs]
        q, ldq, k, v, ldkv = _qkv_cols(projs, C)
        if heads:
            o, lse = ops.attn_heads_fwd(dt, q, ldq, k, v, ldkv, sqk, c_q, scale, M, H, d)
            return o, lse, ("heads", impl, 1.0, scale), (() if lean else tuple(projs))
        route, qpre = "split", 1.0
        dt_in = dt if dt == F32 else BF16_F32IN
        if dp != d:
            *bufs, sqk_a = ops.heads_pad_fwd(dt_in, q, ldq, k, ldkv, v, ldkv, sqk, c_q, B, T, H, d)
        else:
            bufs = ops.qknorm_fwd(dt_in, q, ldq, k, ldkv, v, ldkv, sqk, c_q, B, T, H, d)
        if sqk is None or dp != d:
            del projs, q, k, v
    qh, kh, vh, _, _ = bufs
    o, lse = ops.attn_fwd(dt, impl, qh, kh, vh, scale, sqk_a, c_q, q_prescale=qpre)
    if dp != d:
        o = ops.unpad_cols(o, M, H, d)
    return o, lse, (route, impl, qpre, scale), (() if lean else tuple(bufs))


def _attn_bwd(rt: _Runtime, att, saved, do: Tensor, o: Tensor, lse: Tensor, grads, sqk: Optional[Tensor], c_q: float,
              dims):
    B, T, C, H, d, M = dims
    dt = rt.dt
    route, impl, qpre, scale = att
    dq, lddq, dk, dv, lddkv = _qkv_cols(grads, C)
    if route == "heads":
        q, ldq, k, v, ldkv = _qkv_cols(saved, C)
        return ops.attn_heads_bwd(dt, do, q, ldq, k, v, ldkv, sqk, c_q, scale, lse, dq, lddq, dk, dv, lddkv, M, H,
                                  d), None
    qh, kh, vh, rq, rk = saved
    fused_bwd = (dt != F32 and d == 64) if sqk is not None else route == "fused"
    if fused_bwd:
        return ops.attn_bwd_qknorm(do, qh, kh, vh, o, lse, scale, rq, rk, sqk, c_q, dq, lddq, dk, dv, lddkv,
                                   q_prescale=qpre)
    dp = ops.PAD_HEAD_DIM if d in PADDED_HEAD_DIMS else d
    if dp != d:
        do, o = ops.pad_cols(do, M, H, d), ops.pad_cols(o, M, H, d)
    dqh, dkh, dvh = ops.attn_bwd(dt, impl, do, qh, kh, vh, o, lse, scale)
    del do, o
    merge = ops.heads_pad_bwd if dp != d else ops.qknorm_bwd
    return merge(dt, dqh, dkh, dvh, qh, kh, rq, rk, sqk, c_q, dq, lddq, dk, lddkv, dv, lddkv, B, T, H, d), None


def _swiglu_fwd(rt: _Runtime, A: Tensor, w: str, M: int, F: int, K: int, gs: Optional[Tensor],
                gs_fused: Optional[Tensor], gscale: float, lean: bool = False):
    dt, sh = rt.dt, rt.sh
    bias = sh.get(w + ".b")
    if ops.fusable(dt, M, 2 * F, K):
        if lean:
            return None, ops.gemm_nt_swiglu_act(A, sh[w + ".W"], M, F, K, gs_fused, gscale, bias=bias)
        return ops.gemm_nt_swiglu(A, sh[w + ".W"], M, F, K, gs_fused, gscale, bias=bias)
    uv32 = ops.gemm_nt(A, sh[w + ".W"], M, 2 * F, K, out_dtype=torch.float32, bias=bias)
    x = ops.swiglu_fwd(dt if dt == F32 else BF16_F32IN, uv32, gs, gscale, M, F)
    if lean:
        return None, x
    return (uv32 if dt == F32 else ops.cast(uv32, dt)), x


def _swiglu_bwd(rt: _Runtime, dy: Tensor, w: str, uv: Tensor, M: int, F: int, K: int, gs: Optional[Tensor],
                gscale: float):
    dt, sh = rt.dt, rt.sh
    if ops.fusable(dt, M, F, K):
        return ops.gemm_nt_swiglu_bwd(dy, sh[w + ".Wt"], uv, M, F, K, gs, gscale)
    dx = ops.gemm_nt(dy, sh[w + ".Wt"], M, F, K, out_dtype=ops.tdtype(dt))
    return ops.swiglu_bwd(dt, dx, uv, gs, gscale, M, F)


def _wgrad(rt: _Runtime, dy: Tensor, a: Tensor, params, M: int, N: int, K: int, has_b: bool, perm: int = 0):
    g = ops.gemm_tn(dy, a, rt.grad_buf(params, (N, K)), M, N, K, perm=perm)
    return g, (_bias_grad(dy, M, N, perm) if has_b else None)


class _BlockFn(torch.autograd.Function):

    @staticmethod
    def forward(ctx, x, x_lo, rt, idx, with_skip, impl, skip_param, attn_alpha, mlp_alpha, sqk, suv, wq, wk, wv, wo,
                wfc, wp, bq, bk_, bv, bo, bfc, bp, chained=False, lean=False, gates=None):
        cfg = rt.model.config
        dims = _dims(rt, x.shape[0])
        B, T, C, H, d, M = dims
        dt = rt.dt
        sh = rt.sh
        c_q, c_a = 1.0 / cfg.base_scale, 0.05 / cfg.base_scale
        pre = f"h{idx}."
        has_b = bq is not None
        o, lse, att, att_saved = _attn_fwd(rt, impl, ((x_lo, pre + "qkv", 3),), sqk, c_q, math.sqrt(d), dims,
                                           lean)
        y = ops.gemm_nt(o, sh[pre + "o.W"], M, C, C, out_dtype=rt.y_dtype(), bias=sh.get(pre + "o.b"))
        g_att, g_mlp = gates if gates is not None else (None, None)
        h1, h1_lo = ops.lerp_fwd(dt, x, y, attn_alpha, c_a, want_lo=(dt != F32), gate=g_att)
        if dt == F32:
            h1_lo = h1
        uv, xm = _swiglu_fwd(rt, h1_lo, pre + "fc", M, 4 * C, C, suv, sh[pre + "suv_i"], math.sqrt(C), lean)
        y2 = ops.gemm_nt(xm, sh[pre + "p.W"], M, C, 4 * C, out_dtype=rt.y_dtype(), bias=sh.get(pre + "p.b"))
        if with_skip:
            xn, xn_lo = ops.lerp_fwd(dt, h1, y2, mlp_alpha, c_a, skip_x=x, skip=skip_param, want_lo=(dt != F32),
                                     gate=g_mlp)
        else:
            xn, xn_lo = ops.lerp_fwd(dt, h1, y2, mlp_alpha, c_a, want_lo=(dt != F32), gate=g_mlp)
        if dt == F32:
            xn_lo = xn.new_empty(0)
        if lean:
            return xn, xn_lo
        ctx.rt, ctx.idx, ctx.with_skip, ctx.has_b, ctx.attn = rt, idx, with_skip, has_b, att
        ctx.chained = bool(chained)
        ctx.gates = (g_att, g_mlp)
        ctx.dims = dims
        ctx.par = (skip_param, attn_alpha, mlp_alpha, sqk, suv, wq, wk, wv, wo, wfc, wp)
        ctx.save_for_backward(x, x_lo, o, lse, y, h1, h1_lo, uv, xm, y2, skip_param, attn_alpha, mlp_alpha, sqk, suv,
                              *att_saved)
        ctx.mark_non_differentiable(xn_lo)
        ctx.set_materialize_grads(False)
        return xn, xn_lo

    @staticmethod
    def backward(ctx, dxn, _unused):
        (x, x_lo, o, lse, y, h1, h1_lo, uv, xm, y2, skip_param, attn_alpha, mlp_alpha, sqk, suv,
         *att_saved) = ctx.saved_tensors
        rt, idx = ctx.rt, ctx.idx
        B, T, C, H, d, M = ctx.dims
        p_skip, p_aalpha, p_malpha, p_sqk, p_suv, p_wq, p_wk, p_wv, p_wo, p_wfc, p_wp = ctx.par
        cfg = rt.model.config
        dt, td = rt.dt, ops.tdtype(rt.dt)
        sh = rt.sh
        c_q, c_a = 1.0 / cfg.base_scale, 0.05 / cfg.base_scale
        pre = f"h{idx}."
        if dxn is None:
            return (None,) * 26
        dxn = dxn.contiguous()
        g_att, g_mlp = ctx.gates
        lo_dgrad = dt != F32
        red = ops.ReduceBatch()
        dxn, carry_in = _take_carry(rt, idx, ctx.chained, dxn)
        if ctx.with_skip:
            dh1, _, dy2_lo, dx, part_lam, part_skip = ops.lerp_bwd(dt, dxn, h1, y2, mlp_alpha, c_a, x, skip_param,
                                                                   None, False, False, True, dout_add=carry_in,
                                                                   gate=g_mlp)
            dskip = rt.grad_buf((p_skip,), p_skip.shape)
            red.add(part_skip, dskip, False)
        else:
            dh1, _, dy2_lo, _, part_lam, _ = ops.lerp_bwd(dt, dxn, h1, y2, mlp_alpha, c_a, None, None, None, False,
                                                          False, True, dout_add=carry_in)
            dx, dskip = None, None
        d_mlp_alpha = _param_grad_alpha(rt, part_lam, p_malpha, c_a, red)
        duv, part_suv = _swiglu_bwd(rt, dy2_lo, pre + "p", uv, M, 4 * C, C, suv, math.sqrt(C))
        g_wp, g_bp = _wgrad(rt, dy2_lo, xm, (p_wp,), M, C, 4 * C, ctx.has_b)
        d_suv = _param_grad_scaled(rt, part_suv, p_suv, 1.0, red)
        if lo_dgrad:
            dh1_add = ops.gemm_nt(duv, sh[pre + "fc.Wt"], M, C, 8 * C, out_dtype=td)
        else:
            dh1_add = None
            ops.gemm_nt(duv, sh[pre + "fc.Wt"], M, C, 8 * C, out=dh1, accumulate=True)
        g_wfc, g_bfc = _wgrad(rt, duv, h1_lo, (p_wfc,), M, 8 * C, C, ctx.has_b, perm=1)
        if dx is None:
            dx, _, dy_lo, _, part_lam, _ = ops.lerp_bwd(dt, dh1, x, y, attn_alpha, c_a, None, None, None, False,
                                                        False, True, dout_add=dh1_add)
        else:
            dx, _, dy_lo, _, part_lam, _ = ops.lerp_bwd(dt, dh1, x, y, attn_alpha, c_a, None, None, dx, True, False,
                                                        True, dout_add=dh1_add, gate=g_att)
        d_attn_alpha = _param_grad_alpha(rt, part_lam, p_aalpha, c_a, red)
        do = ops.gemm_nt(dy_lo, sh[pre + "o.Wt"], M, C, C, out_dtype=td)
        g_wo, g_bo = _wgrad(rt, dy_lo, o, (p_wo,), M, C, C, ctx.has_b)
        dqkv = torch.empty((M, 3 * C), device=x.device, dtype=td)
        part_q, part_k = _attn_bwd(rt, ctx.attn, att_saved, do, o, lse, (dqkv,), sqk, c_q, ctx.dims)
        d_sqk = _param_grad_scaled(rt, part_q, p_sqk, c_q, red, part_b=part_k)
        if lo_dgrad and ctx.chained:
            rt.carry = (idx - 1, dx, ops.gemm_nt(dqkv, sh[pre + "qkv.Wt"], M, C, 3 * C, out_dtype=td))
        else:
            ops.gemm_nt(dqkv, sh[pre + "qkv.Wt"], M, C, 3 * C, out=dx, accumulate=True)
        g_qkv, g_bqkv = _wgrad(rt, dqkv, x_lo, (p_wq, p_wk, p_wv), M, 3 * C, C, ctx.has_b)
        red.flush()
        gq, gk, gv = g_qkv[:C], g_qkv[C:2 * C], g_qkv[2 * C:]
        if ctx.has_b:
            gbq, gbk, gbv = g_bqkv[:C], g_bqkv[C:2 * C], g_bqkv[2 * C:]
        else:
            gbq = gbk = gbv = None
        return (dx, None, None, None, None, None, dskip, d_attn_alpha, d_mlp_alpha, d_sqk, d_suv, gq, gk, gv, g_wo,
                g_wfc, g_wp, gbq, gbk, gbv, g_bo, g_bfc, g_bp, None, None, None)


class _CrossFn(torch.autograd.Function):

    @staticmethod
    def forward(ctx, loc, glo, loc_lo, glo_lo, rt, impl, attn_alpha, sqk, wq, wk, wv, wproj, wout, bq, bk_, bv, bproj, bout,
                chained=False, lean=False):
        cfg = rt.model.config
        dims = _dims(rt, loc.shape[0])
        B, T, C, H, d, M = dims
        dt = rt.dt
        sh = rt.sh
        c_q, c_a = 1.0 / cfg.base_scale, 0.05 / cfg.base_scale
        has_b = bq is not None
        if dt == F32:
            loc_lo, glo_lo = loc, glo
        else:
            loc_lo = ops.cast(loc, dt) if loc_lo is None else loc_lo
            glo_lo = ops.cast(glo, dt) if glo_lo is None else glo_lo
        o, lse, att, att_saved = _attn_fwd(rt, impl, ((loc_lo, "x.q", 1), (glo_lo, "x.kv", 2)), sqk, c_q,
                                           math.sqrt(d), dims, lean)
        pr, g = _swiglu_fwd(rt, o, "x.proj", M, C, C, None, None, 1.0, lean)
        y = ops.gemm_nt(g, sh["x.out.W"], M, C, C, out_dtype=rt.y_dtype(), bias=sh.get("x.out.b"))
        x, x_lo = ops.lerp_fwd(dt, loc, y, attn_alpha, c_a, want_lo=(dt != F32))
        if dt == F32:
            x_lo = x.new_empty(0)
        if lean:
            return x, x_lo
        ctx.rt, ctx.has_b, ctx.attn = rt, has_b, att
        ctx.chained = bool(chained)
        ctx.dims = dims
        ctx.par = (attn_alpha, sqk, wq, wk, wv, wproj, wout)
        ctx.save_for_backward(loc, glo, loc_lo, glo_lo, o, lse, pr, g, y, attn_alpha, sqk, *att_saved)
        ctx.mark_non_differentiable(x_lo)
        ctx.set_materialize_grads(False)
        return x, x_lo

    @staticmethod
    def backward(ctx, dx, _unused):
        if dx is None:
            return (None,) * 20
        loc, glo, loc_lo, glo_lo, o, lse, pr, g, y, attn_alpha, sqk, *att_saved = ctx.saved_tensors
        rt = ctx.rt
        B, T, C, H, d, M = ctx.dims
        p_alpha, p_sqk, p_wq, p_wk, p_wv, p_wproj, p_wout = ctx.par
        cfg = rt.model.config
        dt, td = rt.dt, ops.tdtype(rt.dt)
        sh = rt.sh
        dev = loc.device
        c_q, c_a = 1.0 / cfg.base_scale, 0.05 / cfg.base_scale
        dx = dx.contiguous()
        red = ops.ReduceBatch()
        dx, carry_in = _take_carry(rt, -1, ctx.chained, dx)
        dloc, _, dy_lo, _, part_lam, _ = ops.lerp_bwd(dt, dx, loc, y, attn_alpha, c_a, None, None, None,
                                                      False, False, True, dout_add=carry_in)
        d_alpha = _param_grad_alpha(rt, part_lam, p_alpha, c_a, red)
        dpr, _ = _swiglu_bwd(rt, dy_lo, "x.out", pr, M, C, C, None, 1.0)
        g_wout, g_bout = _wgrad(rt, dy_lo, g, (p_wout,), M, C, C, ctx.has_b)
        do = ops.gemm_nt(dpr, sh["x.proj.Wt"], M, C, 2 * C, out_dtype=td)
        g_wproj, g_bproj = _wgrad(rt, dpr, o, (p_wproj,), M, 2 * C, C, ctx.has_b, perm=1)
        dq = torch.empty((M, C), device=dev, dtype=td)
        dkv = torch.empty((M, 2 * C), device=dev, dtype=td)
        part_q, part_k = _attn_bwd(rt, ctx.attn, att_saved, do, o, lse, (dq, dkv), sqk, c_q, ctx.dims)
        d_sqk = _param_grad_scaled(rt, part_q, p_sqk, c_q, red, part_b=part_k)
        ops.gemm_nt(dq, sh["x.q.Wt"], M, C, C, out=dloc, accumulate=True)
        dglo = ops.gemm_nt(dkv, sh["x.kv.Wt"], M, C, 2 * C, out_dtype=torch.float32)
        g_wq, g_bq = _wgrad(rt, dq, loc_lo, (p_wq,), M, C, C, ctx.has_b)
        g_wkv, g_bkv = _wgrad(rt, dkv, glo_lo, (p_wk, p_wv), M, 2 * C, C, ctx.has_b)
        red.flush()
        gbk, gbv = (g_bkv[:C], g_bkv[C:]) if ctx.has_b else (None, None)
        return (dloc, dglo, None, None, None, None, d_alpha, d_sqk, g_wq, g_wkv[:C], g_wkv[C:], g_wproj, g_wout, g_bq, gbk, gbv,
                g_bproj, g_bout, None, None)


class _StdBlockFn(torch.autograd.Function):

    @staticmethod
    def forward(ctx, x, rt, idx, with_skip, want_lo, impl, skip_param, w_att, w_mlp, wq, wk, wv, wo, wfc, wp, bq, bk_,
                bv, bo, bfc, bp, lean=False, gates=None):
        dims = _dims(rt, x.shape[0])
        B, T, C, H, d, M = dims
        dt = rt.dt
        lo = dt != F32
        sh = rt.sh
        pre = f"h{idx}."
        has_b = bq is not None
        a, a_lo, r_att = ops.res_rmsnorm_fwd(dt, x, None, w_att.detach(), RMS_EPS, want_lo=lo)
        if not lo:
            a_lo = a
        o, lse, att, att_saved = _attn_fwd(rt, impl, ((a_lo, pre + "qkv", 3),), None, 0.0, 1.0 / math.sqrt(d),
                                           dims, lean)
        y = ops.gemm_nt(o, sh[pre + "o.W"], M, C, C, out_dtype=rt.y_dtype(), bias=sh.get(pre + "o.b"))
        g_att, g_mlp = gates if gates is not None else (None, None)
        bm, bm_lo, r_mlp = ops.res_rmsnorm_fwd(dt, a, y, w_mlp.detach(), RMS_EPS, want_lo=lo, gate=g_att)
        if not lo:
            bm_lo = bm
        uv, xm = _swiglu_fwd(rt, bm_lo, pre + "fc", M, 4 * C, C, None, None, 1.0, lean)
        if with_skip:
            y2 = ops.gemm_nt(xm, sh[pre + "p.W"], M, C, 4 * C, out_dtype=rt.y_dtype(), bias=sh.get(pre + "p.b"))
            xn, xn_lo = ops.res_skip_fwd(dt, bm, y2, skip_param.detach(), x, want_lo=(lo and want_lo), gate=g_mlp)
        else:
            y2 = ops.gemm_nt(xm, sh[pre + "p.W"], M, C, 4 * C, out_dtype=torch.float32, bias=sh.get(pre + "p.b"),
                             rowadd=bm, rowadd_period=M)
            xn, xn_lo = y2, (ops.cast(y2, dt) if lo and want_lo else None)
        if xn_lo is None:
            xn_lo = xn.new_empty(0)
        if lean:
            return xn, xn_lo
        ctx.rt, ctx.idx, ctx.with_skip, ctx.has_b, ctx.attn = rt, idx, with_skip, has_b, att
        ctx.dims = dims
        ctx.gates = (g_att, g_mlp)
        ctx.par = (skip_param, w_att, w_mlp, wq, wk, wv, wo, wfc, wp)
# ... 852 lines not shown
```

nvit_amd/ops.py:

```python
from __future__ import annotations

import ctypes as C
import math
from typing import Optional, Tuple

import torch

from . import _lib, resample
from ._lib import BF16, F32, check

Tensor = torch.Tensor
MAX_PART_BLOCKS = _lib.const("MAX_PART_BLOCKS")
ROW_WAVES = _lib.const("ROW_WAVES")
ROW_GRID_MAX = _lib.const("ROW_GRID_MAX")
PAD_HEAD_DIM = _lib.const("PAD_HEAD_DIM")
REDUCE_MAX_ITEMS = _lib.const("COLSUM_REDUCE_MAX_ITEMS")
ATTN_BWD_PART_ROWS = _lib.const("ATTN_BWD_PART_ROWS")
SWIGLU_BWD_TILE_ROWS = _lib.const("SWIGLU_BWD_TILE_ROWS")
SWIGLU_BWD_PART_ROWS = _lib.const("SWIGLU_BWD_PART_ROWS")
PATCH_K_STEP = _lib.const("PATCH_EMBED_K_STEP")
PATCH_TILE_ROWS = _lib.const("PATCH_EMBED_TILE_ROWS")
SHADOW_TILE = _lib.const("SHADOW_TILE")


# ... 51 lines not shown

FUSE_MIN_ELEMS = 256 * 256 * 64


def fusable(dt: int, M: int, N: int, K: int) -> bool:
    return bool(_lib.load().nvit_gemm_nt_fusable(dt, M, N, K)) and M * N >= FUSE_MIN_ELEMS


def _chk_fused_bias(bias: Optional[Tensor], n: int, ref: Tensor, what: str) -> None:
    if bias is None:
        return
    if (bias.dtype != torch.float32 or bias.dim() != 1 or bias.numel() != n or not bias.is_contiguous()
            or bias.device != ref.device):
        raise ValueError(f"{what}: bias must be a contiguous fp32 tensor of {n} elements on {ref.device}, got "
                         f"{bias.dtype} {tuple(bias.shape)} stride {bias.stride()} on {bias.device}")


def gemm_nt_swiglu(A: Tensor, B: Tensor, M: int, F: int, K: int, gs: Optional[Tensor], gscale: float, *,
                   bias: Optional[Tensor] = None):
    _chk_dev(A, B)
    _chk_fused_bias(bias, 2 * F, A, "gemm_nt_swiglu")
    uv = torch.empty((M, 2 * F), device=A.device, dtype=torch.bfloat16)
    xm = torch.empty((M, F), device=A.device, dtype=torch.bfloat16)
    check(_lib.load().nvit_gemm_nt_swiglu_bias(dt_of(A), _p(A), A.stride(0), _p(B), B.stride(0), _p(uv), _p(xm), M, F, K,
                                               _p(gs), gscale, _p(bias), _s()), "nvit_gemm_nt_swiglu_bias")
    return uv, xm


def gemm_nt_swiglu_act(A: Tensor, B: Tensor, M: int, F: int, K: int, gs: Optional[Tensor], gscale: float, *,
                       bias: Optional[Tensor] = None) -> Tensor:
    _chk_dev(A, B)
    _chk_fused_bias(bias, 2 * F, A, "gemm_nt_swiglu_act")
    xm = torch.empty((M, F), device=A.device, dtype=torch.bfloat16)
    check(_lib.load().nvit_gemm_nt_swiglu_act_bias(dt_of(A), _p(A), A.stride(0), _p(B), B.stride(0), _p(xm), M, F, K,
                                                   _p(gs), gscale, _p(bias), _s()), "nvit_gemm_nt_swiglu_act_bias")
    return xm


def gemm_nt_swiglu_bwd(A: Tensor, B: Tensor, uv: Tensor, M: int, F: int, K: int, gs: Optional[Tensor], gscale: float):
    _chk_dev(A, B, uv)
    duv = torch.empty((M, 2 * F), device=A.device, dtype=torch.bfloat16)
    part = (torch.empty((round_up(M, SWIGLU_BWD_TILE_ROWS) // SWIGLU_BWD_PART_ROWS, 2 * F), device=A.device,
                        dtype=torch.float32) if gs is not None else None)
    check(_lib.load().nvit_gemm_nt_swiglu_bwd(dt_of(A), _p(A), A.stride(0), _p(B), B.stride(0), _p(uv), _p(duv),
                                              _p(part), M, F, K, _p(gs), gscale, _s()), "nvit_gemm_nt_swiglu_bwd")
    return duv, part


def qk_buffers(dt: int, B: int, T: int, H: int, d: int, device, norm: bool = True):
    td = tdtype(dt)
    qh = torch.empty((B, H, T, d), device=device, dtype=td)
    if not norm:
        return qh, torch.empty_like(qh), torch.empty_like(qh), None, None
    return (qh, torch.empty_like(qh), torch.empty_like(qh),
            torch.empty((B * T, H), device=device, dtype=torch.float32),
            torch.empty((B * T, H), device=device, dtype=torch.float32))


LOG2E = 1.4426950408889634


def attn_q_prescale(d: int) -> float:
    return math.sqrt(d) * LOG2E


def gemm_nt_qknorm(A: Tensor, B: Tensor, M: int, K: int, nparts: int, part0: int, sqk: Optional[Tensor], c_q: float,
                   Bsz: int, T: int, H: int, d: int, bufs=None, q_prescale: float = 1.0, *,
                   bias: Optional[Tensor] = None):
    _chk_dev(A, B)
    _chk_fused_bias(bias, nparts * H * d, A, "gemm_nt_qknorm")
    if bufs is None:
        bufs = qk_buffers(dt_of(A), Bsz, T, H, d, A.device, norm=sqk is not None)
    qh, kh, vh, rq, rk = bufs
    check(_lib.load().nvit_gemm_nt_qknorm_bias(dt_of(A), _p(A), A.stride(0), _p(B), B.stride(0), M, K, nparts, part0,
                                               _p(sqk), c_q, q_prescale, _p(qh), _p(kh), _p(vh), _p(rq), _p(rk), T, H,
                                               d, _p(bias), _s()), "nvit_gemm_nt_qknorm_bias")
    return bufs


_ws_cache = {}


def _workspace(nbytes: int, device) -> Tensor:
    key = (device, torch.cuda.current_stream().cuda_stream)
    ws = _ws_cache.get(key)
    if ws is None or ws.numel() * 4 < nbytes:
        ws = torch.empty(max(nbytes // 4 + 1, 1 << 20), device=device, dtype=torch.float32)
        _ws_cache[key] = ws
    return ws


def tn_splits(Mred: int, N: int, K: int, dt: int) -> int:
    if N % 256 == 0 and K % 256 == 0 and Mred >= 4096:
        tiles = (N // 256) * (K // 256)
        flops = 2.0 * Mred * N * K
        best, best_t = 1, float("inf")
        for s in range(1, 65):
            if Mred // s < 1024:
                break
            items = tiles * s
            eff = items / (math.ceil(items / 256) * 256)
            t = flops / (1.0e15 * eff) + 2.0 * s * N * K * 4 / 4.0e12
            if t < best_t:
                best, best_t = s, t
        return best
    tiles = math.ceil(N / 128) * math.ceil(K / 128)
    rb = bk_of(dt)
    want = max(1, math.ceil(1024 / tiles))
    return max(1, min(want, math.ceil(Mred / (4 * rb)), 64))


def gemm_tn(A: Tensor, B: Tensor, G: Tensor, Mred: int, N: int, K: int, perm: int = 0, accumulate: bool = False,
            lda: Optional[int] = None, ldb: Optional[int] = None, ldg: Optional[int] = None) -> Tensor:
    _chk_dev(A, B, G)
    dt = dt_of(A)
    assert dt_of(B) == dt and G.dtype == torch.float32
    lda = A.stride(0) if lda is None else lda
    ldb = B.stride(0) if ldb is None else ldb
    ldg = G.stride(0) if ldg is None else ldg
    splits = tn_splits(Mred, N, K, dt)
    nbytes = splits * N * K * 4 + 256
    ws = _workspace(nbytes, A.device)
    check(_lib.load().nvit_gemm_tn(dt, _p(A), lda, _p(B), ldb, _p(G), ldg, Mred, N, K, splits, _p(ws),
                                   ws.numel() * 4, perm, int(accumulate), _s()), "nvit_gemm_tn")
    return G


_LERP_BWD_BLOCKS: dict = {}
PART_BLOCKS = 1024
assert PART_BLOCKS <= MAX_PART_BLOCKS


def _row_part_blocks(M: int) -> int:
    return min(PART_BLOCKS, math.ceil(M / ROW_WAVES))


def _part_blocks(nblk: Optional[int], default: int, name: str) -> int:
    if nblk is None:
        return default
    if isinstance(nblk, bool) or not isinstance(nblk, int) or not 1 <= nblk <= MAX_PART_BLOCKS:
        raise ValueError(f"{name}: nblk must be an integer in 1..{MAX_PART_BLOCKS}, got {nblk!r}")
    return nblk


def _chk_gate(gate: Tensor, M: int, ref: Tensor, what: str) -> int:
    if (not isinstance(gate, Tensor) or gate.dtype != torch.float32 or gate.dim() != 1 or not gate.is_contiguous()
            or gate.device != ref.device or gate.numel() < 1 or M % gate.numel()):
        raise ValueError(f"{what}: gate must be a contiguous fp32 vector on {ref.device} whose length divides M={M}")
    return M // gate.numel()


def lerp_fwd(dt: int, h: Tensor, y: Tensor, alpha: Tensor, c_a: float, skip_x: Optional[Tensor] = None,
             skip: Optional[Tensor] = None, want_lo: bool = True, *,
             gate: Optional[Tensor] = None) -> Tuple[Tensor, Optional[Tensor]]:
    M, Cc = h.shape
    out = torch.empty_like(h)
    out_lo = torch.empty((M, Cc), device=h.device, dtype=tdtype(dt)) if want_lo else None
    if gate is not None:
        T = _chk_gate(gate, M, h, "lerp_fwd")
        check(_lib.load().nvit_lerp_fwd_gated(dt, _p(h), _p(y), dt_of(y), _p(alpha), c_a, _p(skip_x), _p(skip), _p(gate),
                                              T, _p(out), _p(out_lo), M, Cc, _s()), "nvit_lerp_fwd_gated")
        return out, out_lo
    check(_lib.load().nvit_lerp_fwd(dt, _p(h), _p(y), dt_of(y), _p(alpha), c_a, _p(skip_x), _p(skip), _p(out),
                                    _p(out_lo), M, Cc, _s()), "nvit_lerp_fwd")
    return out, out_lo


def lerp_bwd(dt: int, dout: Tensor, h: Tensor, y: Tensor, alpha: Tensor, c_a: float, skip_x: Optional[Tensor],
             skip: Optional[Tensor], dh: Optional[Tensor], accum_dh: bool, want_dy_f32: bool, want_dy_lo: bool,
             dout_add: Optional[Tensor] = None, *, nblk: Optional[int] = None, gate: Optional[Tensor] = None):
    if dout_add is not None and (dout_add.dtype != torch.bfloat16 or dout_add.shape != h.shape or not dout_add.is_contiguous()):
        raise ValueError("lerp_bwd: dout_add must be a contiguous bf16 [M,C] tensor")
    M, Cc = h.shape
    dev = h.device
    if dh is None:
        dh = torch.empty_like(h)
        accum_dh = False
    gated = gate is not None
    if gated:
        T = _chk_gate(gate, M, h, "lerp_bwd")
        if (skip_x is not None) == bool(accum_dh):
            raise ValueError("lerp_bwd: the gated kernel takes skip_x without accum_dh, or accum_dh without skip_x")
    key = (dt, dt_of(y), Cc, dout_add is not None, skip_x is not None, bool(accum_dh), gated)
    nres = _LERP_BWD_BLOCKS.get(key)
    if nres is None:
        blocks = _lib.load().nvit_lerp_bwd_gated_blocks if gated else _lib.load().nvit_lerp_bwd_blocks
        nres = int(blocks(dt, dt_of(y), Cc, int(key[3]), int(key[4]), int(key[5]))) or PART_BLOCKS
        _LERP_BWD_BLOCKS[key] = nres
    nblk = _part_blocks(nblk, min(nres, math.ceil(M / ROW_WAVES)), "lerp_bwd")
    dy = torch.empty_like(h) if want_dy_f32 else None
    dy_lo = torch.empty((M, Cc), device=dev, dtype=tdtype(dt)) if want_dy_lo else None
    dskip_x = torch.empty_like(h) if skip_x is not None else None
    part = torch.empty((ROW_WAVES * nblk, Cc), device=dev, dtype=torch.float32)
    pskip = torch.empty((ROW_WAVES * nblk,), device=dev, dtype=torch.float32) if skip_x is not None else None
    if gated:
        check(_lib.load().nvit_lerp_bwd_gated(dt, _p(dout), _p(dout_add), _p(h), _p(y), dt_of(y), _p(alpha), c_a, _p(skip_x),
                                              _p(skip), _p(gate), T, _p(dh), int(accum_dh), _p(dy), _p(dy_lo), _p(dskip_x),
                                              _p(part), _p(pskip), nblk, M, Cc, _s()), "nvit_lerp_bwd_gated")
        return dh, dy, dy_lo, dskip_x, part, pskip
    check(_lib.load().nvit_lerp_bwd(dt, _p(dout), _p(dout_add), _p(h), _p(y), dt_of(y), _p(alpha), c_a, _p(skip_x), _p(skip),
                                    _p(dh), int(accum_dh), _p(dy), _p(dy_lo), _p(dskip_x), _p(part), _p(pskip),
                                    nblk, M, Cc, _s()), "nvit_lerp_bwd")
    return dh, dy, dy_lo, dskip_x, part, pskip


def rmsnorm_fwd(x: Tensor, w: Tensor, eps: float):
    M, Cc = x.shape
    out = torch.empty_like(x)
    rstd = torch.empty((M,), device=x.device, dtype=torch.float32)
    check(_lib.load().nvit_rmsnorm_fwd(_p(x), _p(w), eps, _p(out), _p(rstd), M, Cc, _s()), "nvit_rmsnorm_fwd")
    return out, rstd


def rmsnorm_bwd(dout: Tensor, x: Tensor, w: Tensor, rstd: Tensor, *, nblk: Optional[int] = None):
    M, Cc = x.shape
    nblk = _part_blocks(nblk, _row_part_blocks(M), "rmsnorm_bwd")
    dx = torch.empty_like(x)
    part = torch.empty((nblk, Cc), device=x.device, dtype=torch.float32)
    check(_lib.load().nvit_rmsnorm_bwd(_p(dout), _p(x), _p(w), _p(rstd), _p(dx), _p(part), nblk, M, Cc, _s()),
          "nvit_rmsnorm_bwd")
    dw = torch.empty((Cc,), device=x.device, dtype=torch.float32)
    colsum_reduce(part, dw, False)
    return dx, dw


def _chk_rows(shape, *ts, f32=(), name=""):
    for t in ts + tuple(f32):
        if t is None:
            continue
        _chk_dev(t)
        if not t.is_contiguous():
            raise ValueError(f"{name}: operands must be contiguous")
        if t.dtype not in (torch.float32, torch.bfloat16):
            raise ValueError(f"{name}: fp32 or bf16 operands expected, got {t.dtype}")
    for t in f32:
        if t is not None and t.dtype != torch.float32:
            raise ValueError(f"{name}: fp32 operand expected, got {t.dtype}")
    for t in ts + tuple(f32):
        if t is not None and t.dim() == 2 and tuple(t.shape) != tuple(shape):
            raise ValueError(f"{name}: operand of shape {tuple(t.shape)}, expected {tuple(shape)}")


def _chk_vec(C: int, *vs, name=""):
    for v in vs:
        _chk_dev(v)
        if v.dtype != torch.float32 or not v.is_contiguous() or v.numel() != C:
            raise ValueError(f"{name}: contiguous fp32 vector of {C} elements expected")


def res_rmsnorm_fwd(dt: int, a: Tensor, y: Optional[Tensor], w: Tensor, eps: float, want_lo: bool = True, *,
                    gate: Optional[Tensor] = None):
    M, Cc = a.shape
    _chk_rows((M, Cc), y, f32=(a,), name="res_rmsnorm_fwd")
    _chk_vec(Cc, w, name="res_rmsnorm_fwd")
    out = torch.empty_like(a)
    out_lo = torch.empty((M, Cc), device=a.device, dtype=tdtype(dt)) if want_lo else None
    rstd = torch.empty((M,), device=a.device, dtype=torch.float32)
    if gate is not None:
        if y is None:
            raise ValueError("res_rmsnorm_fwd: a gate needs the branch output y")
        T = _chk_gate(gate, M, a, "res_rmsnorm_fwd")
        check(_lib.load().nvit_res_rmsnorm_fwd_gated(dt, _p(a), _p(y), dt_of(y), _p(w), eps, _p(gate), T, _p(out), _p(out_lo),
                                                     _p(rstd), M, Cc, _s()), "nvit_res_rmsnorm_fwd_gated")
        return out, out_lo, rstd
    check(_lib.load().nvit_res_rmsnorm_fwd(dt, _p(a), _p(y), dt_of(y) if y is not None else F32, _p(w), eps, _p(out),
                                           _p(out_lo), _p(rstd), M, Cc, _s()), "nvit_res_rmsnorm_fwd")
    return out, out_lo, rstd


def res_rmsnorm_bwd(dt: int, g: Tensor, a: Tensor, y: Optional[Tensor], w: Tensor, rstd: Tensor,
                    g_add: Optional[Tensor] = None, dz: Optional[Tensor] = None, want_lo: bool = False, *,
                    nblk: Optional[int] = None, gate: Optional[Tensor] = None):
    M, Cc = a.shape
    _chk_rows((M, Cc), y, g_add, f32=(a, g, dz), name="res_rmsnorm_bwd")
    _chk_vec(Cc, w, name="res_rmsnorm_bwd")
    _chk_vec(M, rstd, name="res_rmsnorm_bwd")
    if g_add is not None and g_add.dtype != tdtype(dt):
        raise ValueError("res_rmsnorm_bwd: g_add must be a contiguous [M,C] tensor of the mode's operand type")
    accum = dz is not None
    if dz is None:
        dz = torch.empty_like(a)
    nblk = _part_blocks(nblk, _row_part_blocks(M), "res_rmsnorm_bwd")
    dz_lo = torch.empty((M, Cc), device=a.device, dtype=tdtype(dt)) if want_lo else None
    part = torch.empty((ROW_WAVES * nblk, Cc), device=a.device, dtype=torch.float32)
    if gate is not None:
        if y is None or g_add is None:
            raise ValueError("res_rmsnorm_bwd: the gated kernel needs the branch output y and the addend g_add")
        T = _chk_gate(gate, M, a, "res_rmsnorm_bwd")
        check(_lib.load().nvit_res_rmsnorm_bwd_gated(dt, _p(g), _p(g_add), _p(a), _p(y), dt_of(y), _p(w), _p(rstd), _p(gate),
                                                     T, _p(dz), int(accum), _p(dz_lo), _p(part), nblk, M, Cc, _s()),
              "nvit_res_rmsnorm_bwd_gated")
        return dz, dz_lo, part
    check(_lib.load().nvit_res_rmsnorm_bwd(dt, _p(g), _p(g_add), _p(a), _p(y), dt_of(y) if y is not None else F32, _p(w),
                                           _p(rstd), _p(dz), int(accum), _p(dz_lo), _p(part), nblk, M, Cc, _s()),
          "nvit_res_rmsnorm_bwd")
    return dz, dz_lo, part


def res_skip_fwd(dt: int, h: Tensor, y: Tensor, skip: Tensor, x: Tensor, want_lo: bool = True, *,
                 gate: Optional[Tensor] = None):
    M, Cc = h.shape
    _chk_rows((M, Cc), y, f32=(h, x), name="res_skip_fwd")
    _chk_vec(1, skip, name="res_skip_fwd")
    out = torch.empty_like(h)
    out_lo = torch.empty((M, Cc), device=h.device, dtype=tdtype(dt)) if want_lo else None
    if gate is not None:
        T = _chk_gate(gate, M, h, "res_skip_fwd")
        check(_lib.load().nvit_res_skip_fwd_gated(dt, _p(h), _p(y), dt_of(y), _p(skip), _p(x), _p(gate), T, _p(out),
                                                  _p(out_lo), M, Cc, _s()), "nvit_res_skip_fwd_gated")
        return out, out_lo
    check(_lib.load().nvit_res_skip_fwd(dt, _p(h), _p(y), dt_of(y), _p(skip), _p(x), _p(out), _p(out_lo), M, Cc, _s()),
          "nvit_res_skip_fwd")
    return out, out_lo


def res_skip_bwd(dt: int, dout: Tensor, h: Tensor, y: Tensor, skip: Tensor, x: Tensor, want_lo: bool = True, *,
                 nblk: Optional[int] = None, gate: Optional[Tensor] = None):
    M, Cc = h.shape
    _chk_rows((M, Cc), y, f32=(dout, h, x), name="res_skip_bwd")
    _chk_vec(1, skip, name="res_skip_bwd")
    nblk = _part_blocks(nblk, _row_part_blocks(M), "res_skip_bwd")
    dh = torch.empty_like(h)
    dx = torch.empty_like(h)
    dh_lo = torch.empty((M, Cc), device=h.device, dtype=tdtype(dt)) if want_lo else None
    part = torch.empty((ROW_WAVES * nblk,), device=h.device, dtype=torch.float32)
    if gate is not None:
        T = _chk_gate(gate, M, h, "res_skip_bwd")
        check(_lib.load().nvit_res_skip_bwd_gated(dt, _p(dout), _p(h), _p(y), dt_of(y), _p(skip), _p(x), _p(gate), T, _p(dh),
                                                  _p(dh_lo), _p(dx), _p(part), nblk, M, Cc, _s()), "nvit_res_skip_bwd_gated")
        return dh, dh_lo, dx, part
    check(_lib.load().nvit_res_skip_bwd(dt, _p(dout), _p(h), _p(y), dt_of(y), _p(skip), _p(x), _p(dh), _p(dh_lo), _p(dx),
                                        _p(part), nblk, M, Cc, _s()), "nvit_res_skip_bwd")
    return dh, dh_lo, dx, part


def norm_skip_fwd(src: Tensor, tgt: Optional[Tensor], skip: Tensor) -> Tensor:
    M, Cc = src.shape
    out = torch.empty_like(src)
    check(_lib.load().nvit_norm_skip_fwd(_p(src), _p(tgt), _p(skip), _p(out), M, Cc, _s()), "nvit_norm_skip_fwd")
    return out


def norm_skip_bwd(dout: Tensor, src: Tensor, tgt: Optional[Tensor], skip: Tensor, *, nblk: Optional[int] = None):
    M, Cc = src.shape
    nblk = _part_blocks(nblk, _row_part_blocks(M), "norm_skip_bwd")
    dsrc = torch.empty_like(src)
    dtgt = torch.empty_like(src) if tgt is not None else None
    part = torch.empty((nblk,), device=src.device, dtype=torch.float32)
    check(_lib.load().nvit_norm_skip_bwd(_p(dout), _p(src), _p(tgt), _p(skip), _p(dsrc), _p(dtgt), _p(part), nblk, M,
                                         Cc, _s()), "nvit_norm_skip_bwd")
    dskip = torch.empty_like(skip)
    colsum_reduce(part, dskip, False)
    return dsrc, dtgt, dskip


def _pad_out(out, shape, dtype, device, name: str) -> Tensor:
    if out is None:
        return torch.empty(shape, device=device, dtype=dtype)
# ... 657 lines not shown
```

Measured before the change: 1281 images/sec.

## Recompute attention lerp inside the MLP lerp kernels instead of storing f32 h1

The f32 h1 output of the attention lerp is no longer written or saved when the skip path runs in bf16 without gates. The second lerp (forward and backward) reads x and the bf16 attention output and recomputes h1 in registers, which removes one f32 [M,C] write and two f32 reads per block. The new kernels also use a swizzle-based wave reduction and higher occupancy launch bounds. The cost is extra arithmetic, extra register pressure and one extra bf16 read per pass.

Result: no change. 1285 images/sec, median of 6 (+0.3%).

```diff
diff --git a/include/nvit_hip.h b/include/nvit_hip.h
--- a/include/nvit_hip.h
+++ b/include/nvit_hip.h
@@ -125,6 +125,14 @@
                   float c_a, const float* skip_x, const float* skip, float* dh, int accum_dh, float* dy,
                   void* dy_lo, float* dskip_x, float* part_dlam, float* part_dskip, int nblk, int M, int C,
                   void* stream);
+int nvit_lerp_fwd_chain(int dt, const float* x, const void* y_att, const float* attn_alpha, const void* y2,
+                        const float* mlp_alpha, float c_a, const float* skip, float* out, void* out_lo, int M, int C,
+                        void* stream);
+int nvit_lerp_bwd_chain_blocks(int dt, int C, int has_add);
+int nvit_lerp_bwd_chain(int dt, const float* dout, const void* dout_add, const float* x, const void* y_att,
+                        const float* attn_alpha, const void* y2, const float* mlp_alpha, float c_a, const float* skip,
+                        float* dh, void* dy_lo, float* dskip_x, float* part_dlam, float* part_dskip, int nblk, int M,
+                        int C, void* stream);
 int nvit_lerp_fwd_gated(int dt, const float* h, const void* y, int y_dt, const float* alpha, float c_a,
                         const float* skip_x, const float* skip, const float* gate, int rows_per_sample, float* out,
                         void* out_lo, int M, int C, void* stream);
diff --git a/nvit_amd/_lib.py b/nvit_amd/_lib.py
--- a/nvit_amd/_lib.py
+++ b/nvit_amd/_lib.py
@@ -75,6 +75,9 @@
     "nvit_lerp_fwd": [_i, _vp, _vp, _i, _vp, _f, _vp, _vp, _vp, _vp, _i, _i, _vp],
     "nvit_lerp_bwd_blocks": [_i, _i, _i, _i, _i, _i],
     "nvit_lerp_bwd": [_i, _vp, _vp, _vp, _vp, _i, _vp, _f, _vp, _vp, _vp, _i, _vp, _vp, _vp, _vp, _vp, _i, _i, _i, _vp],
+    "nvit_lerp_fwd_chain": [_i, _vp, _vp, _vp, _vp, _vp, _f, _vp, _vp, _vp, _i, _i, _vp],
+    "nvit_lerp_bwd_chain_blocks": [_i, _i, _i],
+    "nvit_lerp_bwd_chain": [_i, _vp, _vp, _vp, _vp, _vp, _vp, _vp, _f, _vp, _vp, _vp, _vp, _vp, _vp, _i, _i, _i, _vp],
     "nvit_lerp_fwd_gated": [_i, _vp, _vp, _i, _vp, _f, _vp, _vp, _vp, _i, _vp, _vp, _i, _i, _vp],
     "nvit_lerp_bwd_gated_blocks": [_i, _i, _i, _i, _i, _i],
     "nvit_lerp_bwd_gated": [_i, _vp, _vp, _vp, _vp, _i, _vp, _f, _vp, _vp, _vp, _i, _vp, _i, _vp, _vp, _vp, _vp, _vp, _i, _i,
diff --git a/nvit_amd/csrc/rowops.hip b/nvit_amd/csrc/rowops.hip
--- a/nvit_amd/csrc/rowops.hip
+++ b/nvit_amd/csrc/rowops.hip
@@ -26,12 +26,26 @@
     if (c < C) store4<T>(p + c, r.v[i]);
   }
 }
-template <int NV>
+template <bool LEAN>
+__device__ __forceinline__ float wave_sum_as(float v) {
+  if constexpr (!LEAN) return wave_sum(v);
+  v += __shfl_xor(v, 32, 64);
+#define NVIT_SWZ_XOR(o_) v += __int_as_float(__builtin_amdgcn_ds_swizzle(__float_as_int(v), ((o_) << 10) | 0x1f))
+  NVIT_SWZ_XOR(16);
+  NVIT_SWZ_XOR(8);
+  NVIT_SWZ_XOR(4);
+  NVIT_SWZ_XOR(2);
+  NVIT_SWZ_XOR(1);
+#undef NVIT_SWZ_XOR
+  return v;
+}
+
+template <int NV, bool LEAN = false>
 __device__ __forceinline__ float row_dot(const RowVec<NV>& a, const RowVec<NV>& b) {
   float s = 0.f;
 #pragma unroll
   for (int i = 0; i < NV; ++i) s += a.v[i][0] * b.v[i][0] + a.v[i][1] * b.v[i][1] + a.v[i][2] * b.v[i][2] + a.v[i][3] * b.v[i][3];
-  return wave_sum(s);
+  return wave_sum_as<LEAN>(s);
 }
 
 template <int NV>
@@ -55,6 +69,8 @@
   int M, C;
   const float* gate;
   int T;
+  const void* y0;
+  const float* alpha0;
 };
 
 __device__ __forceinline__ float row_gate(const float* gate, int m, int T) {
@@ -62,61 +78,120 @@
   return ((cfloat_p)gate)[__builtin_amdgcn_readfirstlane(m) / T];
 }
 
-template <int NV, typename TY, typename TL, bool GATED>
-__global__ __launch_bounds__(256) void lerp_fwd_kernel(LerpFwdArgs a) {
-  const int lane = threadIdx.x & 63, wid = threadIdx.x >> 6;
-  RowVec<NV> lam;
-  row_load<NV, float>(lam, a.alpha, a.C, lane);
+__device__ __forceinline__ int wave_id_uniform() { return __builtin_amdgcn_readfirstlane(threadIdx.x >> 6); }
+
+template <int NV, typename TY>
+struct RowRaw {
+  std::conditional_t<sizeof(TY) == 2, uint2, f32x4> v[NV];
+};
+template <int NV, typename TY, bool NT>
+__device__ __forceinline__ void row_load_raw(RowRaw<NV, TY>& r, const TY* p, int C, int lane) {
+#pragma unroll
+  for (int i = 0; i < NV; ++i) {
+    const int c = (i * 64 + lane) * 4;
+    if constexpr (sizeof(TY) == 2) {
+      typedef unsigned int u32x2_ __attribute__((ext_vector_type(2)));
+      const u32x2_* q = reinterpret_cast<const u32x2_*>(p + c);
+      r.v[i] = c < C ? __builtin_bit_cast(uint2, NT ? __builtin_nontemporal_load(q) : *q) : make_uint2(0u, 0u);
+    } else {
+      const f32x4* q = reinterpret_cast<const f32x4*>(p + c);
+      r.v[i] = c < C ? (NT ? __builtin_nontemporal_load(q) : *q) : (f32x4){0.f, 0.f, 0.f, 0.f};
+    }
+  }
+}
+__device__ __forceinline__ f32x4 unpack4(uint2 raw) {
+  const bf16x4 b4 = __builtin_bit_cast(bf16x4, raw);
+  return (f32x4){(float)b4[0], (float)b4[1], (float)b4[2], (float)b4[3]};
+}
+__device__ __forceinline__ f32x4 unpack4(f32x4 raw) { return raw; }
+template <int NV, bool LEAN = false, typename TY>
+__device__ __forceinline__ float row_dot(const RowRaw<NV, TY>& a, const RowRaw<NV, TY>&) {
+  float s = 0.f;
+#pragma unroll
+  for (int i = 0; i < NV; ++i) {
+    const f32x4 u = unpack4(a.v[i]);
+    s += u[0] * u[0] + u[1] * u[1] + u[2] * u[2] + u[3] * u[3];
+  }
+  return wave_sum_as<LEAN>(s);
+}
+template <int NV, typename TY>
+__device__ __forceinline__ void row_unpack(RowVec<NV>& y, const RowRaw<NV, TY>& r) {
+#pragma unroll
+  for (int i = 0; i < NV; ++i) y.v[i] = unpack4(r.v[i]);
+}
+
+__device__ __forceinline__ f32x4 lerp_mix(const f32x4& av, const f32x4& lam, const f32x4& bv) { return av + lam * (bv - av); }
+
+template <int NV, bool GATED, bool LEAN = false, typename YRow>
+__device__ __forceinline__ void lerp_row(RowVec<NV>& r, const RowVec<NV>& x, const YRow& y, const RowVec<NV>& lam,
+                                         float gt) {
+  const float rsx = 1.0f / sqrtf(row_dot<NV, LEAN>(x, x));
+  const float rsy = 1.0f / sqrtf(row_dot<NV, LEAN>(y, y));
+#pragma unroll
+  for (int i = 0; i < NV; ++i) {
+    const f32x4 av = x.v[i] * rsx, bv = unpack4(y.v[i]) * rsy;
+    if constexpr (GATED) r.v[i] = lerp_mix(av, lam.v[i] * gt, bv);
+    else r.v[i] = lerp_mix(av, lam.v[i], bv);
+  }
+  const float rsr = 1.0f / sqrtf(row_dot<NV, LEAN>(r, r));
+#pragma unroll
+  for (int i = 0; i < NV; ++i) r.v[i] = r.v[i] * rsr;
+}
+
+template <int NV>
+__device__ __forceinline__ void abs_steps(RowVec<NV>& lam, float c_a) {
 #pragma unroll
   for (int i = 0; i < NV; ++i)
 #pragma unroll
-    for (int e = 0; e < 4; ++e) lam.v[i][e] = fabsf(lam.v[i][e] * a.c_a);
-  const float skip = a.skip_x ? a.skip[0] : 0.f;
+    for (int e = 0; e < 4; ++e) lam.v[i][e] = fabsf(lam.v[i][e] * c_a);
+}
+template <int NV>
+__device__ __forceinline__ void abs_steps(RowVec<NV>& lam, const float* alpha, float c_a, int C, int lane) {
+  row_load<NV, float>(lam, alpha, C, lane);
+  abs_steps<NV>(lam, c_a);
+}
+
+template <int NV, typename TY, typename TL, bool GATED, bool CHAIN = false>
+__global__ __launch_bounds__(256, CHAIN && NV <= 3 ? 6 : 1) void lerp_fwd_kernel(LerpFwdArgs a) {
+  static_assert(!(GATED && CHAIN), "the chained kernel is not gated");
+  const int lane = threadIdx.x & 63, wid = CHAIN ? wave_id_uniform() : threadIdx.x >> 6;
+  RowVec<NV> lam, lam0;
+  abs_steps<NV>(lam, a.alpha, a.c_a, a.C, lane);
+  if constexpr (CHAIN) abs_steps<NV>(lam0, a.alpha0, a.c_a, a.C, lane);
+  const bool with_skip = CHAIN || a.skip_x;
+  const float skip = with_skip ? a.skip[0] : 0.f;
   for (int m = blockIdx.x * ROW_WAVES + wid; m < a.M; m += gridDim.x * ROW_WAVES) {
     RowVec<NV> x, y, r, xs;
-    row_load_f32_nt<NV>(x, a.h + (size_t)m * a.C, a.C, lane);
-#pragma unroll
-    for (int i = 0; i < NV; ++i) {
-      const int c = (i * 64 + lane) * 4;
-      if constexpr (sizeof(TY) == 2) {
-        uint2 raw = make_uint2(0u, 0u);
-        if (c < a.C) {
-          typedef unsigned int u32x2_ __attribute__((ext_vector_type(2)));
-          raw = __builtin_bit_cast(uint2, __builtin_nontemporal_load(reinterpret_cast<const u32x2_*>(reinterpret_cast<const TY*>(a.y) + (size_t)m * a.C + c)));
-        }
-        const bf16x4 b4 = __builtin_bit_cast(bf16x4, raw);
-        y.v[i] = (f32x4){(float)b4[0], (float)b4[1], (float)b4[2], (float)b4[3]};
-      } else {
-        y.v[i] = c < a.C ? __builtin_nontemporal_load(reinterpret_cast<const f32x4*>(reinterpret_cast<const float*>(a.y) + (size_t)m * a.C + c)) : (f32x4){0.f, 0.f, 0.f, 0.f};
-      }
-    }
-    if (a.skip_x) row_load_f32_nt<NV>(xs, a.skip_x + (size_t)m * a.C, a.C, lane);
+    RowRaw<NV, TY> yr, y0r;
+    const size_t ro = (size_t)m * a.C;
+    row_load_f32_nt<NV>(x, a.h + ro, a.C, lane);
+    row_load_raw<NV, TY, true>(yr, reinterpret_cast<const TY*>(a.y) + ro, a.C, lane);
+    if constexpr (CHAIN) row_load_raw<NV, TY, true>(y0r, reinterpret_cast<const TY*>(a.y0) + ro, a.C, lane);
+    else if (a.skip_x) row_load_f32_nt<NV>(xs, a.skip_x + ro, a.C, lane);
     float gt = 1.0f;
     if constexpr (GATED) gt = row_gate(a.gate, m, a.T);
-    const float rsx = 1.0f / sqrtf(row_dot<NV>(x, x));
-    const float rsy = 1.0f / sqrtf(row_dot<NV>(y, y));
-#pragma unroll
-    for (int i = 0; i < NV; ++i) {
-      const f32x4 av = x.v[i] * rsx, bv = y.v[i] * rsy;
-      if constexpr (GATED) r.v[i] = av + (lam.v[i] * gt) * (bv - av);
-      else r.v[i] = av + lam.v[i] * (bv - av);
-    }
-    const float rsr = 1.0f / sqrtf(row_dot<NV>(r, r));
-#pragma unroll
-    for (int i = 0; i < NV; ++i) r.v[i] = r.v[i] * rsr;
-    if (a.skip_x) {
+    if constexpr (CHAIN) {
+      xs = x;
+      row_unpack<NV, TY>(y, y0r);
+      lerp_row<NV, false>(x, xs, y, lam0, 1.0f);
+    }
+    row_unpack<NV, TY>(y, yr);
+    lerp_row<NV, GATED>(r, x, y, lam, gt);
+    if (with_skip) {
 #pragma unroll
       for (int i = 0; i < NV; ++i) r.v[i] = r.v[i] * skip + xs.v[i];
       const float rst = 1.0f / sqrtf(row_dot<NV>(r, r));
 #pragma unroll
       for (int i = 0; i < NV; ++i) r.v[i] = r.v[i] * rst;
     }
-#pragma unroll
-    for (int i = 0; i < NV; ++i) {
-      const int c = (i * 64 + lane) * 4;
-      if (c < a.C) __builtin_nontemporal_store(r.v[i], reinterpret_cast<f32x4*>(a.out + (size_t)m * a.C + c));
-    }
-    if (a.out_lo) row_store<NV, TL>(r, reinterpret_cast<TL*>(a.out_lo) + (size_t)m * a.C, a.C, lane);
+    if (a.out) {
+#pragma unroll
+      for (int i = 0; i < NV; ++i) {
+        const int c = (i * 64 + lane) * 4;
+        if (c < a.C) __builtin_nontemporal_store(r.v[i], reinterpret_cast<f32x4*>(a.out + ro + c));
+      }
+    }
+    if (a.out_lo) row_store<NV, TL>(r, reinterpret_cast<TL*>(a.out_lo) + ro, a.C, lane);
   }
 }
 
@@ -139,6 +214,8 @@
   int M, C;
   const float* gate;
   int T;
+  const void* y0;
+  const float* alpha0;
 };
 
 template <int NV>
@@ -146,25 +223,30 @@
   return a[0] * b[0] + a[1] * b[1] + a[2] * b[2] + a[3] * b[3];
 }
 
-template <int NV, typename TY, typename TL, bool ADD, bool SKIP, bool ACCUM, bool GATED>
-__global__ __launch_bounds__(256, 1) void lerp_bwd_kernel(LerpBwdArgs a) {
-  const int lane = threadIdx.x & 63, wid = threadIdx.x >> 6;
+template <int NV, typename TY, typename TL, bool ADD, bool SKIP, bool ACCUM, bool GATED, bool CHAIN = false>
+__global__ __launch_bounds__(256, CHAIN && NV <= 3 ? 4 : 1) void lerp_bwd_kernel(LerpBwdArgs a) {
+  static_assert(!CHAIN || (SKIP && !ACCUM && !GATED), "the chained kernel is the ungated MLP half");
+  const int lane = threadIdx.x & 63, wid = CHAIN ? wave_id_uniform() : threadIdx.x >> 6;
   RowVec<NV> lam, dlam;
-  row_load<NV, float>(lam, a.alpha, a.C, lane);
-#pragma unroll
-  for (int i = 0; i < NV; ++i) {
-    dlam.v[i] = (f32x4){0.f, 0.f, 0.f, 0.f};
-#pragma unroll
-    for (int e = 0; e < 4; ++e) lam.v[i][e] = fabsf(lam.v[i][e] * a.c_a);
-  }
+  abs_steps<NV>(lam, a.alpha, a.c_a, a.C, lane);
+#pragma unroll
+  for (int i = 0; i < NV; ++i) dlam.v[i] = (f32x4){0.f, 0.f, 0.f, 0.f};
   const float skip = SKIP ? a.skip[0] : 0.f;
   float dskip_acc = 0.f;
   for (int m = blockIdx.x * ROW_WAVES + wid; m < a.M; m += gridDim.x * ROW_WAVES) {
     RowVec<NV> av, bv, g, t, old;
     uint2 ga[NV];
+    RowRaw<NV, TY> y0r, yr;
+    RowVec<NV> lam0;
     const size_t ro = (size_t)m * a.C;
-    row_load_f32_nt<NV>(av, a.h + ro, a.C, lane);
-    row_load<NV, TY>(bv, reinterpret_cast<const TY*>(a.y) + ro, a.C, lane);
+    if constexpr (CHAIN) {
+      row_load_raw<NV, TY, false>(y0r, reinterpret_cast<const TY*>(a.y0) + ro, a.C, lane);
+      row_load_raw<NV, TY, false>(yr, reinterpret_cast<const TY*>(a.y) + ro, a.C, lane);
+      row_load<NV, float>(lam0, a.alpha0, a.C, lane);
+    } else {
+      row_load_f32_nt<NV>(av, a.h + ro, a.C, lane);
+      row_load<NV, TY>(bv, reinterpret_cast<const TY*>(a.y) + ro, a.C, lane);
+    }
     row_load_f32_nt<NV>(g, a.dout + ro, a.C, lane);
     if constexpr (ADD) {
 #pragma unroll
@@ -184,19 +266,24 @@
         g.v[i] += (f32x4){(float)q[0], (float)q[1], (float)q[2], (float)q[3]};
       }
     }
-    const float rsx = 1.0f / sqrtf(row_dot<NV>(av, av));
-    const float rsy = 1.0f / sqrtf(row_dot<NV>(bv, bv));
+    if constexpr (CHAIN) {
+      abs_steps<NV>(lam0, a.c_a);
+      lerp_row<NV, false, true>(av, t, y0r, lam0, 1.0f);
+      row_unpack<NV, TY>(bv, yr);
+    }
+    const float rsx = 1.0f / sqrtf(row_dot<NV, CHAIN>(av, av));
+    const float rsy = 1.0f / sqrtf(row_dot<NV, CHAIN>(bv, bv));
     if constexpr (ACCUM) row_load<NV, float>(old, a.dh + ro, a.C, lane);
     float ss = 0.f;
 #pragma unroll
     for (int i = 0; i < NV; ++i) {
       av.v[i] = av.v[i] * rsx;
       bv.v[i] = bv.v[i] * rsy;
-      const f32x4 ou = av.v[i] + NVIT_LAM(i) * (bv.v[i] - av.v[i]);
+      const f32x4 ou = lerp_mix(av.v[i], NVIT_LAM(i), bv.v[i]);
       ss += dot4<NV>(ou, ou);
     }
-    const float rsr = 1.0f / sqrtf(wave_sum(ss));
-#define NVIT_LERP_O(i_) ((av.v[i_] + NVIT_LAM(i_) * (bv.v[i_] - av.v[i_])) * rsr)
+    const float rsr = 1.0f / sqrtf(wave_sum_as<CHAIN>(ss));
+#define NVIT_LERP_O(i_) (lerp_mix(av.v[i_], NVIT_LAM(i_), bv.v[i_]) * rsr)
     if constexpr (SKIP) {
       float st = 0.f;
 #pragma unroll
@@ -204,14 +291,14 @@
         t.v[i] = NVIT_LERP_O(i) * skip + t.v[i];
         st += dot4<NV>(t.v[i], t.v[i]);
       }
-      const float rst = 1.0f / sqrtf(wave_sum(st));
+      const float rst = 1.0f / sqrtf(wave_sum_as<CHAIN>(st));
       float tg = 0.f;
 #pragma unroll
       for (int i = 0; i < NV; ++i) {
         t.v[i] = t.v[i] * rst;
         tg += dot4<NV>(t.v[i], g.v[i]);
       }
-      tg = wave_sum(tg);
+      tg = wave_sum_as<CHAIN>(tg);
       float dso = 0.f;
 #pragma unroll
       for (int i = 0; i < NV; ++i) {
@@ -219,14 +306,14 @@
         dso += dot4<NV>(g.v[i], NVIT_LERP_O(i));
       }
       row_store<NV, float>(g, a.dskip_x + ro, a.C, lane);
-      dskip_acc += wave_sum(dso);
+      dskip_acc += wave_sum_as<CHAIN>(dso);
 #pragma unroll
       for (int i = 0; i < NV; ++i) g.v[i] = g.v[i] * skip;
     }
     float og = 0.f;
 #pragma unroll
     for (int i = 0; i < NV; ++i) og += dot4<NV>(NVIT_LERP_O(i), g.v[i]);
-    og = wave_sum(og);
+    og = wave_sum_as<CHAIN>(og);
     float ada = 0.f, bdb = 0.f;
 #pragma unroll
     for (int i = 0; i < NV; ++i) {
@@ -237,8 +324,8 @@
       bdb += dot4<NV>(bv.v[i], db);
     }
 #undef NVIT_LERP_O
-    ada = wave_sum(ada);
-    bdb = wave_sum(bdb);
+    ada = wave_sum_as<CHAIN>(ada);
+    bdb = wave_sum_as<CHAIN>(bdb);
 #pragma unroll
     for (int i = 0; i < NV; ++i) {
       const int c = (i * 64 + lane) * 4;
@@ -1048,9 +1135,11 @@
   return f(type_tag<float>{}, type_tag<bf16>{});
 }
 
-static auto lerp_bwd_select(int C, int y_dt, int dt, bool has_add, bool has_skip, bool accum) -> void (*)(LerpBwdArgs) {
+static auto lerp_bwd_select(int C, int y_dt, int dt, bool has_add, bool has_skip, bool accum, bool chain = false)
+    -> void (*)(LerpBwdArgs) {
   return with_row_types(C, y_dt, dt, [&](auto nv, auto ty, auto tl) {
     return with_bool(has_add, [&](auto add) {
+      if (chain) return &lerp_bwd_kernel<nv, bf16, bf16, add, true, false, false, true>;
       return with_bool(has_skip, [&](auto skip) {
         return with_bool(accum, [&](auto acc) {
           return &lerp_bwd_kernel<nv, tag_t<decltype(ty)>, tag_t<decltype(tl)>, add, skip, acc, false>;
@@ -1080,15 +1169,31 @@
                              void* stream) {
   NVIT_REQUIRE(C % 4 == 0 && C <= NVIT_MAX_EMBD && M > 0, "lerp_fwd: C=%d must be a multiple of 4 and <= %d", C, NVIT_MAX_EMBD);
   NVIT_REQUIRE(!skip_x || skip, "lerp_fwd: skip_x without skip");
+  NVIT_REQUIRE(out || out_lo, "lerp_fwd: neither out nor out_lo");
   LerpFwdArgs a{h, y, alpha, c_a, skip_x, skip, out, out_lo, M, C, nullptr, 1};
   hipStream_t s = (hipStream_t)stream;
   const int grid = row_grid(M);
-  ProfScope ps(NVIT_KID_ROWOPS, 0.0, (double)M * C * (skip_x ? 16.0 : 12.0), s);
+  ProfScope ps(NVIT_KID_ROWOPS, 0.0, (double)M * C * ((skip_x ? 16.0 : 12.0) - (out ? 0.0 : 4.0)), s);
   const auto kernel = with_row_types(C, y_dt, dt, [](auto nv, auto ty, auto tl) {
     return &lerp_fwd_kernel<nv, tag_t<decltype(ty)>, tag_t<decltype(tl)>, false>;
   });
   launch(kernel, dim3(grid), dim3(256), 0, s, a);
   NVIT_CHECK_LAUNCH("lerp_fwd");
+  return NVIT_OK;
+}
+
+extern "C" int nvit_lerp_fwd_chain(int dt, const float* x, const void* y_att, const float* attn_alpha, const void* y2,
+                                   const float* mlp_alpha, float c_a, const float* skip, float* out, void* out_lo, int M,
+                                   int C, void* stream) {
+  NVIT_REQUIRE(C % 4 == 0 && C <= NVIT_MAX_EMBD && M > 0, "lerp_fwd_chain: C=%d must be a multiple of 4 and <= %d", C, NVIT_MAX_EMBD);
+  NVIT_REQUIRE(dt != NVIT_F32, "lerp_fwd_chain: built for the bf16 modes (bf16 y rows and twin)");
+  NVIT_REQUIRE(x && y_att && attn_alpha && y2 && mlp_alpha && skip && out, "lerp_fwd_chain: missing operand");
+  LerpFwdArgs a{x, y2, mlp_alpha, c_a, nullptr, skip, out, out_lo, M, C, nullptr, 1, y_att, attn_alpha};
+  hipStream_t s = (hipStream_t)stream;
+  ProfScope ps(NVIT_KID_ROWOPS, 0.0, (double)M * C * 14.0, s);
+  const auto kernel = with_row_vecs<8>(C, [](auto nv) { return &lerp_fwd_kernel<nv, bf16, bf16, false, true>; });
+  launch(kernel, dim3(row_grid(M)), dim3(256), 0, s, a);
+  NVIT_CHECK_LAUNCH("lerp_fwd_chain");
   return NVIT_OK;
 }
 
@@ -1119,6 +1224,13 @@
   if (C % 4 != 0 || C <= 0 || C > NVIT_MAX_EMBD) return 0;
   const int n = resident_blocks(lerp_bwd_select(C, y_dt, dt, has_add, has_skip, accum));
   return n > NVIT_MAX_PART_BLOCKS ? NVIT_MAX_PART_BLOCKS : n;
+}
+
+extern "C" int nvit_lerp_bwd_chain_blocks(int dt, int C, int has_add) {
+  if (C % 4 != 0 || C <= 0 || C > NVIT_MAX_EMBD || dt == NVIT_F32) return 0;
+  const int own = resident_blocks(lerp_bwd_select(C, NVIT_BF16, dt, has_add, true, false, true));
+  const int unchained = nvit_lerp_bwd_blocks(dt, NVIT_BF16, C, has_add, 1, 0);
+  return own < unchained ? own : unchained;
 }
 
 extern "C" int nvit_lerp_bwd_gated_blocks(int dt, int y_dt, int C, int has_add, int has_skip, int accum) {
@@ -1141,6 +1253,24 @@
   ProfScope ps(NVIT_KID_ROWOPS, 0.0, lb_bytes, s);
   launch(lerp_bwd_select(C, y_dt, dt, dout_add != nullptr, skip_x != nullptr, accum_dh != 0), dim3(nblk), dim3(256), 0, s, a);
   NVIT_CHECK_LAUNCH("lerp_bwd");
+  return NVIT_OK;
+}
+
+extern "C" int nvit_lerp_bwd_chain(int dt, const float* dout, const void* dout_add, const float* x, const void* y_att,
+                                   const float* attn_alpha, const void* y2, const float* mlp_alpha, float c_a,
+                                   const float* skip, float* dh, void* dy_lo, float* dskip_x, float* part_dlam,
+                                   float* part_dskip, int nblk, int M, int C, void* stream) {
+  NVIT_REQUIRE(C % 4 == 0 && C <= NVIT_MAX_EMBD && M > 0, "lerp_bwd_chain: C=%d must be a multiple of 4 and <= %d", C, NVIT_MAX_EMBD);
+  NVIT_REQUIRE(nblk > 0 && nblk <= NVIT_MAX_PART_BLOCKS, "lerp_bwd_chain: nblk out of range");
+  NVIT_REQUIRE(dt != NVIT_F32, "lerp_bwd_chain: built for the bf16 modes (bf16 y rows and dy_lo)");
+  NVIT_REQUIRE(dout && x && y_att && attn_alpha && y2 && mlp_alpha && skip && dh && dskip_x && part_dlam && part_dskip,
+               "lerp_bwd_chain: missing operand");
+  LerpBwdArgs a{dout, (const bf16*)dout_add, nullptr, y2, mlp_alpha, c_a, x, skip, dh, 0, nullptr, dy_lo, dskip_x, part_dlam, part_dskip, M, C, nullptr, 1, y_att, attn_alpha};
+  hipStream_t s = (hipStream_t)stream;
+  const double lb_bytes = (double)M * C * (20.0 + (dy_lo ? 2.0 : 0.0) + (dout_add ? 2.0 : 0.0));
+  ProfScope ps(NVIT_KID_ROWOPS, 0.0, lb_bytes, s);
+  launch(lerp_bwd_select(C, NVIT_BF16, dt, dout_add != nullptr, true, false, true), dim3(nblk), dim3(256), 0, s, a);
+  NVIT_CHECK_LAUNCH("lerp_bwd_chain");
   return NVIT_OK;
 }
 
diff --git a/nvit_amd/model.py b/nvit_amd/model.py
--- a/nvit_amd/model.py
+++ b/nvit_amd/model.py
@@ -347,12 +347,15 @@
                                            lean)
         y = ops.gemm_nt(o, sh[pre + "o.W"], M, C, C, out_dtype=rt.y_dtype(), bias=sh.get(pre + "o.b"))
         g_att, g_mlp = gates if gates is not None else (None, None)
-        h1, h1_lo = ops.lerp_fwd(dt, x, y, attn_alpha, c_a, want_lo=(dt != F32), gate=g_att)
+        chain = with_skip and dt != F32 and gates is None
+        h1, h1_lo = ops.lerp_fwd(dt, x, y, attn_alpha, c_a, want_lo=(dt != F32), gate=g_att, want_out=not chain)
         if dt == F32:
             h1_lo = h1
         uv, xm = _swiglu_fwd(rt, h1_lo, pre + "fc", M, 4 * C, C, suv, sh[pre + "suv_i"], math.sqrt(C), lean)
         y2 = ops.gemm_nt(xm, sh[pre + "p.W"], M, C, 4 * C, out_dtype=rt.y_dtype(), bias=sh.get(pre + "p.b"))
-        if with_skip:
+        if chain:
+            xn, xn_lo = ops.lerp_fwd_chain(dt, x, y, attn_alpha, y2, mlp_alpha, c_a, skip_param)
+        elif with_skip:
             xn, xn_lo = ops.lerp_fwd(dt, h1, y2, mlp_alpha, c_a, skip_x=x, skip=skip_param, want_lo=(dt != F32),
                                      gate=g_mlp)
         else:
@@ -366,16 +369,19 @@
         ctx.gates = (g_att, g_mlp)
         ctx.dims = dims
         ctx.par = (skip_param, attn_alpha, mlp_alpha, sqk, suv, wq, wk, wv, wo, wfc, wp)
-        ctx.save_for_backward(x, x_lo, o, lse, y, h1, h1_lo, uv, xm, y2, skip_param, attn_alpha, mlp_alpha, sqk, suv,
-                              *att_saved)
+        ctx.chain_h1 = chain
+        ctx.save_for_backward(x, x_lo, o, lse, y, *(() if chain else (h1,)), h1_lo, uv, xm, y2, skip_param, attn_alpha,
+                              mlp_alpha, sqk, suv, *att_saved)
         ctx.mark_non_differentiable(xn_lo)
         ctx.set_materialize_grads(False)
         return xn, xn_lo
 
     @staticmethod
     def backward(ctx, dxn, _unused):
-        (x, x_lo, o, lse, y, h1, h1_lo, uv, xm, y2, skip_param, attn_alpha, mlp_alpha, sqk, suv,
-         *att_saved) = ctx.saved_tensors
+        saved = list(ctx.saved_tensors)
+        if ctx.chain_h1:
+            saved.insert(5, None)
+        (x, x_lo, o, lse, y, h1, h1_lo, uv, xm, y2, skip_param, attn_alpha, mlp_alpha, sqk, suv, *att_saved) = saved
         rt, idx = ctx.rt, ctx.idx
         B, T, C, H, d, M = ctx.dims
         p_skip, p_aalpha, p_malpha, p_sqk, p_suv, p_wq, p_wk, p_wv, p_wo, p_wfc, p_wp = ctx.par
@@ -392,9 +398,13 @@
         red = ops.ReduceBatch()
         dxn, carry_in = _take_carry(rt, idx, ctx.chained, dxn)
         if ctx.with_skip:
-            dh1, _, dy2_lo, dx, part_lam, part_skip = ops.lerp_bwd(dt, dxn, h1, y2, mlp_alpha, c_a, x, skip_param,
-                                                                   None, False, False, True, dout_add=carry_in,
-                                                                   gate=g_mlp)
+            if ctx.chain_h1:
+                dh1, dy2_lo, dx, part_lam, part_skip = ops.lerp_bwd_chain(dt, dxn, x, y, attn_alpha, y2, mlp_alpha, c_a,
+                                                                          skip_param, dout_add=carry_in)
+            else:
+                dh1, _, dy2_lo, dx, part_lam, part_skip = ops.lerp_bwd(dt, dxn, h1, y2, mlp_alpha, c_a, x, skip_param,
+                                                                       None, False, False, True, dout_add=carry_in,
+                                                                       gate=g_mlp)
             dskip = rt.grad_buf((p_skip,), p_skip.shape)
             red.add(part_skip, dskip, False)
         else:
diff --git a/nvit_amd/ops.py b/nvit_amd/ops.py
--- a/nvit_amd/ops.py
+++ b/nvit_amd/ops.py
@@ -227,9 +227,11 @@
 
 def lerp_fwd(dt: int, h: Tensor, y: Tensor, alpha: Tensor, c_a: float, skip_x: Optional[Tensor] = None,
              skip: Optional[Tensor] = None, want_lo: bool = True, *,
-             gate: Optional[Tensor] = None) -> Tuple[Tensor, Optional[Tensor]]:
+             gate: Optional[Tensor] = None, want_out: bool = True) -> Tuple[Optional[Tensor], Optional[Tensor]]:
     M, Cc = h.shape
-    out = torch.empty_like(h)
+    if not want_out and (gate is not None or not want_lo):
+        raise ValueError("lerp_fwd: want_out=False needs want_lo and no gate")
+    out = torch.empty_like(h) if want_out else None
     out_lo = torch.empty((M, Cc), device=h.device, dtype=tdtype(dt)) if want_lo else None
     if gate is not None:
         T = _chk_gate(gate, M, h, "lerp_fwd")
@@ -279,6 +281,49 @@
     return dh, dy, dy_lo, dskip_x, part, pskip
 
 
+def _chk_chain(dt: int, x: Tensor, y_att: Tensor, y2: Tensor, what: str) -> None:
+    if dt == F32:
+        raise ValueError(f"{what}: the chained kernels are built for the bf16 modes")
+    for y in (y_att, y2):
+        if y.dtype != torch.bfloat16 or y.shape != x.shape or not y.is_contiguous():
+            raise ValueError(f"{what}: y_att and y2 must be contiguous bf16 [M,C] tensors")
+
+
+def lerp_fwd_chain(dt: int, x: Tensor, y_att: Tensor, attn_alpha: Tensor, y2: Tensor, mlp_alpha: Tensor, c_a: float,
+                   skip: Tensor, want_lo: bool = True) -> Tuple[Tensor, Optional[Tensor]]:
+    _chk_chain(dt, x, y_att, y2, "lerp_fwd_chain")
+    M, Cc = x.shape
+    out = torch.empty_like(x)
+    out_lo = torch.empty((M, Cc), device=x.device, dtype=tdtype(dt)) if want_lo else None
+    check(_lib.load().nvit_lerp_fwd_chain(dt, _p(x), _p(y_att), _p(attn_alpha), _p(y2), _p(mlp_alpha), c_a, _p(skip),
+                                          _p(out), _p(out_lo), M, Cc, _s()), "nvit_lerp_fwd_chain")
+    return out, out_lo
+
+
+def lerp_bwd_chain(dt: int, dout: Tensor, x: Tensor, y_att: Tensor, attn_alpha: Tensor, y2: Tensor, mlp_alpha: Tensor,
+                   c_a: float, skip: Tensor, dout_add: Optional[Tensor] = None, *, nblk: Optional[int] = None):
+    _chk_chain(dt, x, y_att, y2, "lerp_bwd_chain")
+    if dout_add is not None and (dout_add.dtype != torch.bfloat16 or dout_add.shape != x.shape or not dout_add.is_contiguous()):
+        raise ValueError("lerp_bwd_chain: dout_add must be a contiguous bf16 [M,C] tensor")
+    M, Cc = x.shape
+    dev = x.device
+    key = ("chain", dt, Cc, dout_add is not None)
+    nres = _LERP_BWD_BLOCKS.get(key)
+    if nres is None:
+        nres = int(_lib.load().nvit_lerp_bwd_chain_blocks(dt, Cc, int(key[3]))) or PART_BLOCKS
+        _LERP_BWD_BLOCKS[key] = nres
+    nblk = _part_blocks(nblk, min(nres, math.ceil(M / ROW_WAVES)), "lerp_bwd_chain")
+    dh = torch.empty_like(x)
+    dy_lo = torch.empty((M, Cc), device=dev, dtype=tdtype(dt))
+    dskip_x = torch.empty_like(x)
+    part = torch.empty((ROW_WAVES * nblk, Cc), device=dev, dtype=torch.float32)
+    pskip = torch.empty((ROW_WAVES * nblk,), device=dev, dtype=torch.float32)
+    check(_lib.load().nvit_lerp_bwd_chain(dt, _p(dout), _p(dout_add), _p(x), _p(y_att), _p(attn_alpha), _p(y2),
+                                          _p(mlp_alpha), c_a, _p(skip), _p(dh), _p(dy_lo), _p(dskip_x), _p(part),
+                                          _p(pskip), nblk, M, Cc, _s()), "nvit_lerp_bwd_chain")
+    return dh, dy_lo, dskip_x, part, pskip
+
+
 def rmsnorm_fwd(x: Tensor, w: Tensor, eps: float):
     M, Cc = x.shape
     out = torch.empty_like(x)
```
